# Ruslan361/iterative_solvers

Hardware: AMD Instinct MI355X
Metric: cg_iters_per_sec (higher is better)
Workload: dtype f64; 1 GPU; 4096x4096 L-shaped Dirichlet Poisson fp64, matrix-free CG, fixed 2641 iterations; n=4096, unknowns=12574721, rule=rel2

## Files before the change

### include/mi355cg.h

```cpp
#ifndef MI355CG_H
#define MI355CG_H

#include <stddef.h>

#ifdef __cplusplus
extern "C" {
#endif

#define MI355CG_OK            0
#define MI355CG_ERR_INVALID   1
#define MI355CG_ERR_HIP       2
#define MI355CG_ERR_STATE     3

#define MI355CG_F64           0
#define MI355CG_F32_MIXED     1

#define MI355CG_RULE_MSG_MAXNORM  0
#define MI355CG_RULE_REL_2NORM    1

#define MI355CG_STOP_ITERATIONS   0
#define MI355CG_STOP_PRECISION    1
#define MI355CG_STOP_RESIDUAL     2
#define MI355CG_STOP_EXACT_ERROR  3
#define MI355CG_STOP_INTERRUPTED  4
// ... 48 lines not shown
int  mi355cg_set_rhs(mi355cg_handle h, const double *b);
int  mi355cg_setup_on_device(mi355cg_handle h);

int  mi355cg_apply(mi355cg_handle h, const double *x, double *y);
int  mi355cg_apply_device(mi355cg_handle h, const double *x_dev, double *y_dev);

void mi355cg_default_params(mi355cg_params *p, int rule);
int  mi355cg_solve(mi355cg_handle h, const mi355cg_params *params,
                   mi355cg_iter_cb cb, void *user, const volatile int *stop_flag,
                   mi355cg_results *out);
int  mi355cg_get_solution(mi355cg_handle h, double *x);
int  mi355cg_get_recursive_residual(mi355cg_handle h, double *r);
int  mi355cg_get_true_residual(mi355cg_handle h, double *ax_minus_b);

#define MI355CG_PRECOND_NONE    0
#define MI355CG_PRECOND_MG      1
#define MI355CG_PRECOND_MG_ANY  2
int  mi355cg_set_preconditioner(mi355cg_handle h, int kind);
int  mi355cg_apply_preconditioner(mi355cg_handle h, const double *r, double *z);
int  mi355cg_mg_levels(int n, int *levels, int *coarsest_n);
int  mi355cg_mg_hierarchy(int kind, int n, int max_levels, int *levels, int *level_n);

#define MI355CG_CYCLE_F64 0
#define MI355CG_CYCLE_F32 1
int  mi355cg_set_preconditioner_ex(mi355cg_handle h, int kind, int cycle);
int  mi355cg_preconditioner_info(mi355cg_handle h, int *kind, int *cycle, int *levels);

#define MI355CG_SMOOTHER_JACOBI    0
#define MI355CG_SMOOTHER_LINE_X    1
#define MI355CG_SMOOTHER_LINE_Y    2
#define MI355CG_SMOOTHER_LINE_AUTO 3
int  mi355cg_set_smoother(mi355cg_handle h, int smoother);
int  mi355cg_get_smoother(mi355cg_handle h, int *smoother, int *direction);

#define MI355CG_BATCH_MAX 64
int  mi355cg_solve_batch(mi355cg_handle h, const mi355cg_params *params, int nrhs, const double *b, double *x,
                         const volatile int *stop_flag, mi355cg_results *out);
int  mi355cg_solve_batch_device(mi355cg_handle h, const mi355cg_params *params, int nrhs, const double *b_dev, double *x_dev,
                                const volatile int *stop_flag, mi355cg_results *out);
int  mi355cg_batch_release(mi355cg_handle h);

int  mi355cg_set_initial_guess(mi355cg_handle h, const double *x0);
int  mi355cg_set_initial_guess_device(mi355cg_handle h, const double *x0_dev);
int  mi355cg_use_solution_as_initial_guess(mi355cg_handle h);
int  mi355cg_solve_batch_from(mi355cg_handle h, const mi355cg_params *params, int nrhs, const double *b, double *x,
                              const volatile int *stop_flag, mi355cg_results *out);
int  mi355cg_solve_batch_device_from(mi355cg_handle h, const mi355cg_params *params, int nrhs, const double *b_dev, double *x_dev,
                                     const volatile int *stop_flag, mi355cg_results *out);

int  mi355cg_set_shift(mi355cg_handle h, double sigma);
int  mi355cg_get_shift(mi355cg_handle h, double *sigma);
int  mi355cg_time_steps(mi355cg_handle h, const mi355cg_params *params, double tau, double theta, int nsteps,
                        const volatile int *stop_flag, mi355cg_results *out , int *steps_done);
int  mi355cg_get_solution_device(mi355cg_handle h, double *x_dev);

#define MI355CG_EIG_BLOCK_MAX 16
#define MI355CG_EIG_CONVERGED   0
#define MI355CG_EIG_ITERATIONS  1
#define MI355CG_EIG_INTERRUPTED 2
#define MI355CG_EIG_BREAKDOWN   3
typedef struct mi355cg_eig_results {
    int iterations;
    int converged;
    int stop_reason;
    int p_drops;
    double solve_seconds;
} mi355cg_eig_results;
int  mi355cg_eigs(mi355cg_handle h, int nev, int block, double tol, int max_iterations, double *x, double *lambda, double *resid,
                  const volatile int *stop_flag, mi355cg_eig_results *out);
int  mi355cg_eigs_device(mi355cg_handle h, int nev, int block, double tol, int max_iterations, double *x_dev, double *lambda,
                         double *resid, const volatile int *stop_flag, mi355cg_eig_results *out);
int  mi355cg_eigs_release(mi355cg_handle h);
int  mi355cg_block_gram(mi355cg_handle h, int na, const double *a, int nb, const double *b, double *c);
int  mi355cg_block_gram_indexed(mi355cg_handle h, int na, const double *a, int nia, const int *ia, int nb, const double *b,
                                int nib, const int *ib, double *c);
int  mi355cg_block_combine(mi355cg_handle h, int k, const double *s, int m, const double *coef, double *y);
int  mi355cg_rayleigh_ritz(int k, const double *g, const double *hmat, double *theta, double *coef);

int  mi355cg_set_profiling(mi355cg_handle h, int enable);
int  mi355cg_get_kernel_time(mi355cg_handle h, int kernel, double *avg_ms, long long *launches);
int  mi355cg_get_layout(mi355cg_handle h, long long *padded_len, int *pitch_bottom, int *pitch_upper,
                        int *grid_stencil, int *grid_update, int *rows_per_item);
int  mi355cg_get_xfold(mi355cg_handle h, int *depth, int *extra_buffers);

#define MI355CG_SOLVE_LAUNCHES 0
#define MI355CG_SOLVE_ONCHIP   1
int  mi355cg_set_solve_mode(mi355cg_handle h, int mode);
int  mi355cg_get_solve_mode(mi355cg_handle h, int *mode, long long *onchip_launches_last_solve);
int  mi355cg_onchip_plan(int n, int *threads, int *lds_bytes, int *elems_per_thread);

#define MI355CG_MANY_MAX 65536
int  mi355cg_solve_many(mi355cg_handle h, const mi355cg_params *params, int nsys, const double *b, double *x, const double *sigma,
                        const volatile int *stop_flag, mi355cg_results *out);
int  mi355cg_solve_many_from(mi355cg_handle h, const mi355cg_params *params, int nsys, const double *b, double *x, const double *sigma,
                             const volatile int *stop_flag, mi355cg_results *out);
int  mi355cg_solve_many_device(mi355cg_handle h, const mi355cg_params *params, int nsys, const double *b_dev, double *x_dev,
                               const double *sigma_dev, const volatile int *stop_flag, mi355cg_results *out);
int  mi355cg_solve_many_device_from(mi355cg_handle h, const mi355cg_params *params, int nsys, const double *b_dev, double *x_dev,
                                    const double *sigma_dev, const volatile int *stop_flag, mi355cg_results *out);
int  mi355cg_solve_many_info(mi355cg_handle h, int nsys, int *lds_bytes_per_workgroup, int *workgroups_per_cu, long long *workspace_bytes);

int  mi355cg_slab_rows(int n, int world, int rank, int *y_lo, int *y_hi);
int  mi355cg_create_part(int n, int m, double a, double b, double c, double d, int dtype, int device,
                         int y_lo, int y_hi, int x_lo, int x_hi, mi355cg_handle *out);
int  mi355cg_checksum(mi355cg_handle h, int which, double *out2);
int  mi355cg_create_slab(int n, int m, double a, double b, double c, double d, int dtype, int device,
                         int y_lo, int y_hi, mi355cg_handle *out);
int  mi355cg_owned_range(mi355cg_handle h, long long *packed_begin, long long *packed_len, int *y_lo, int *y_hi);
int  mi355cg_dist_begin(mi355cg_handle h, const mi355cg_params *params, void *stream);
int  mi355cg_dist_reduce(mi355cg_handle h, int which , int with_rows, void *stream);
int  mi355cg_dist_sums_ptr(mi355cg_handle h, int which, void **dev_ptr, int *count );
int  mi355cg_dist_record_layout(mi355cg_handle h, int *header, int *row_slot, int *width);
int  mi355cg_dist_scatter_ghosts(mi355cg_handle h, int vector ,
                                 const double *gathered_records, int nranks, int rank, void *stream);
int  mi355cg_dist_stencil(mi355cg_handle h, const double *gathered_update_sums, int nranks, int estride,
                          int rows , void *stream);
int  mi355cg_dist_flip(mi355cg_handle h);
int  mi355cg_dist_update(mi355cg_handle h, const double *gathered_stencil_sums, int nranks, int estride,
                         int rows , void *stream);
int  mi355cg_dist_update_reads_ghosts(mi355cg_handle h);
int  mi355cg_dist_check(mi355cg_handle h, const double *gathered_update_sums, int nranks, int estride, void *stream);
int  mi355cg_dist_summary(mi355cg_handle h, mi355cg_results *out, int *done);
int  mi355cg_dist_finish(mi355cg_handle h, void *stream);
int  mi355cg_dist_history(mi355cg_handle h, int iteration, double *precision, double *residual, double *error);
int  mi355cg_dist_halo(mi355cg_handle h, int vector ,
                       void **send_lo, void **recv_lo, long long *n_send_lo,
                       void **send_hi, void **recv_hi, long long *n_send_hi);
int  mi355cg_dist_halo_recv_counts(mi355cg_handle h, long long *n_from_lo, long long *n_from_hi);

#define MI355CG_DECOMP_ROWS 0
#define MI355CG_DECOMP_2D   1
typedef struct mi355cg_team_s *mi355cg_team;
typedef struct mi355cg_halo_msg {
    int id;
    int peer;
    int send;
    int kind;
    int y0, y1, x0, x1;
    long long count;
} mi355cg_halo_msg;
int  mi355cg_decompose(int n, int world, int decomp, int rank, int *y_lo, int *y_hi, int *x_lo, int *x_hi);
int  mi355cg_halo_plan(int n, int world, int decomp, int rank, int max_msgs, int *n_msgs, mi355cg_halo_msg *msgs);
int  mi355cg_debug_plan(int n, int world, int decomp, int rank, int which, int *n_panels, int *panels,
                        int *grid, int *n_items, int *cls);
int  mi355cg_team_create_local(int n, int m, double a, double b, double c, double d, int world,
                               const int *devices, int ndevices, int decomp, mi355cg_team *out);
int  mi355cg_team_unique_id(void *id128);
int  mi355cg_team_create_rccl(int n, int m, double a, double b, double c, double d, int world, int rank, int device,
                              const void *id128, int decomp, mi355cg_team *out);
void mi355cg_team_destroy(mi355cg_team t);
int  mi355cg_team_solve(mi355cg_team t, const mi355cg_params *params, mi355cg_iter_cb cb, void *user,
                        const volatile int *stop_flag, mi355cg_results *out);
int  mi355cg_team_info(mi355cg_team t, int *world, int *nlocal, int *decomp, long long *size);
int  mi355cg_team_describe(mi355cg_team t, char *buf, int len);
int  mi355cg_team_part(mi355cg_team t, int local_index, mi355cg_handle *part, int *rank);
int  mi355cg_team_get_vector(mi355cg_team t, int which, double *global_packed);
int  mi355cg_team_checksum(mi355cg_team t, int which, double *out2);
int  mi355cg_team_set_vector(mi355cg_team t, int which, const double *global_packed);
int  mi355cg_team_set_dtype(mi355cg_team t, int dtype);
int  mi355cg_team_setup_on_device(mi355cg_team t);
int  mi355cg_team_set_profiling(mi355cg_team t, int enable);
int  mi355cg_team_phase_times(mi355cg_team t, double *kernel_ms, double *comm_ms, double *wall_ms);

#ifdef __cplusplus
}
#endif
// ... 2 lines not shown
```

### iterative_solvers_amd/_capi.py

```python
from __future__ import annotations

import ctypes as C
import os

import numpy as np

from . import build as _build

OK, ERR_INVALID, ERR_HIP, ERR_STATE = 0, 1, 2, 3
F64, F32_MIXED = 0, 1
RULE_MSG_MAXNORM, RULE_REL_2NORM = 0, 1
STOP_ITERATIONS, STOP_PRECISION, STOP_RESIDUAL, STOP_EXACT_ERROR, STOP_INTERRUPTED = range(5)

EXPORTS = [
    "mi355cg_create", "mi355cg_create_csr", "mi355cg_set_true_solution", "mi355cg_destroy", "mi355cg_last_error", "mi355cg_version", "mi355cg_size",
    "mi355cg_get_rhs", "mi355cg_get_true_solution", "mi355cg_get_node_coords", "mi355cg_set_rhs",
    "mi355cg_apply", "mi355cg_apply_device", "mi355cg_default_params", "mi355cg_solve",
    "mi355cg_get_solution", "mi355cg_get_recursive_residual", "mi355cg_get_true_residual",
    "mi355cg_set_profiling", "mi355cg_get_kernel_time", "mi355cg_get_layout",
    "mi355cg_slab_rows", "mi355cg_create_slab", "mi355cg_owned_range", "mi355cg_dist_begin",
    "mi355cg_dist_reduce", "mi355cg_dist_sums_ptr", "mi355cg_dist_record_layout", "mi355cg_dist_scatter_ghosts", "mi355cg_dist_stencil", "mi355cg_dist_flip",
    "mi355cg_dist_update", "mi355cg_dist_update_reads_ghosts", "mi355cg_dist_check", "mi355cg_dist_summary", "mi355cg_dist_finish", "mi355cg_dist_history",
    "mi355cg_dist_halo", "mi355cg_dist_halo_recv_counts",
    "mi355cg_create_part", "mi355cg_checksum", "mi355cg_decompose", "mi355cg_halo_plan",
    "mi355cg_team_create_local", "mi355cg_team_unique_id", "mi355cg_team_create_rccl", "mi355cg_team_destroy",
    "mi355cg_team_solve", "mi355cg_team_info", "mi355cg_team_part", "mi355cg_team_get_vector", "mi355cg_team_set_vector", "mi355cg_team_checksum",
    "mi355cg_team_set_profiling", "mi355cg_team_phase_times", "mi355cg_team_describe", "mi355cg_setup_on_device", "mi355cg_team_setup_on_device", "mi355cg_debug_plan",
    "mi355cg_team_set_dtype", "mi355cg_set_preconditioner", "mi355cg_apply_preconditioner", "mi355cg_mg_levels",
    "mi355cg_mg_hierarchy", "mi355cg_set_preconditioner_ex", "mi355cg_preconditioner_info",
    "mi355cg_solve_batch", "mi355cg_solve_batch_device", "mi355cg_batch_release", "mi355cg_get_xfold",
    "mi355cg_set_initial_guess", "mi355cg_set_initial_guess_device", "mi355cg_use_solution_as_initial_guess",
    "mi355cg_solve_batch_from", "mi355cg_solve_batch_device_from",
    "mi355cg_set_shift", "mi355cg_get_shift", "mi355cg_time_steps", "mi355cg_get_solution_device",
    "mi355cg_eigs", "mi355cg_eigs_device", "mi355cg_eigs_release", "mi355cg_block_gram", "mi355cg_block_gram_indexed",
    "mi355cg_block_combine", "mi355cg_rayleigh_ritz",
    "mi355cg_set_smoother", "mi355cg_get_smoother",
    "mi355cg_set_solve_mode", "mi355cg_get_solve_mode", "mi355cg_onchip_plan",
    "mi355cg_solve_many", "mi355cg_solve_many_from", "mi355cg_solve_many_device", "mi355cg_solve_many_device_from", "mi355cg_solve_many_info",
]
DECOMP_ROWS, DECOMP_2D = 0, 1
PRECOND_NONE, PRECOND_MG, PRECOND_MG_ANY = 0, 1, 2
CYCLE_F64, CYCLE_F32 = 0, 1
SOLVE_LAUNCHES, SOLVE_ONCHIP = 0, 1
SMOOTHER_JACOBI, SMOOTHER_LINE_X, SMOOTHER_LINE_Y, SMOOTHER_LINE_AUTO = 0, 1, 2, 3
BATCH_MAX = 64
MANY_MAX = 65536
EIG_BLOCK_MAX = 16
EIG_BASIS_MAX = 48
EIG_CONVERGED, EIG_ITERATIONS, EIG_INTERRUPTED, EIG_BREAKDOWN = range(4)


class Params(C.Structure):
    _fields_ = [("rule", C.c_int), ("max_iterations", C.c_int),
                ("eps_precision", C.c_double), ("eps_residual", C.c_double),
                ("eps_exact_error", C.c_double), ("eps_rel", C.c_double),
                ("use_true_solution", C.c_int), ("callback_every", C.c_int),
                ("diagnostics", C.c_int), ("sync_every", C.c_int), ("fixed_iterations", C.c_int),
                ("inner_eps", C.c_double)]


class Results(C.Structure):
    _fields_ = [("iterations", C.c_int), ("converged", C.c_int), ("stop_reason", C.c_int),
                ("final_residual_norm", C.c_double), ("final_precision", C.c_double),
                ("final_error_norm", C.c_double), ("r_norm2", C.c_double),
                ("initial_r_norm2", C.c_double), ("solve_seconds", C.c_double),
                ("refine_true_rel", C.c_double), ("refine_outer", C.c_int), ("loop_seconds", C.c_double)]


class EigResults(C.Structure):
    _fields_ = [("iterations", C.c_int), ("converged", C.c_int), ("stop_reason", C.c_int), ("p_drops", C.c_int),
                ("solve_seconds", C.c_double)]


class HaloMsg(C.Structure):
    _fields_ = [("id", C.c_int), ("peer", C.c_int), ("send", C.c_int), ("kind", C.c_int),
                ("y0", C.c_int), ("y1", C.c_int), ("x0", C.c_int), ("x1", C.c_int), ("count", C.c_longlong)]


ITER_CB = C.CFUNCTYPE(None, C.c_void_p, C.c_int, C.c_double, C.c_double, C.c_double)
_DP = np.ctypeslib.ndpointer(dtype=np.float64, flags="C_CONTIGUOUS")

_lib = None


class Mi355cgError(RuntimeError):
    def __init__(self, code: int, text: str):
        super().__init__(f"mi355cg error {code}: {text}")
        self.code = code


def lib_path() -> str:
    return _build.LIB_PATH


def load():
    global _lib
    if _lib is not None:
        return _lib
    path = os.environ.get("MI355CG_LIB") or _build.LIB_PATH
    if path == _build.LIB_PATH and _build.needs_build():
        try:
            _build.build()
        except Exception as e:
            if not os.path.exists(path):
                raise RuntimeError(f"libmi355cg.so is missing and could not be built: {e}") from e
    try:
        import torch
    except ImportError:
        pass
    L = C.CDLL(path)
    H = C.c_void_p
    L.mi355cg_create.argtypes = [C.c_int, C.c_int] + [C.c_double] * 4 + [C.c_int, C.c_int, C.POINTER(H)]
    _IPn = np.ctypeslib.ndpointer(dtype=np.int32, flags="C_CONTIGUOUS")
# ... 18 lines not shown
    L.mi355cg_get_kernel_time.argtypes = [H, C.c_int, C.POINTER(C.c_double), C.POINTER(C.c_longlong)]
    L.mi355cg_get_layout.argtypes = [H, C.POINTER(C.c_longlong)] + [C.POINTER(C.c_int)] * 5
    LLP, IP, VPP = C.POINTER(C.c_longlong), C.POINTER(C.c_int), C.POINTER(C.c_void_p)
    L.mi355cg_slab_rows.argtypes = [C.c_int, C.c_int, C.c_int, IP, IP]
    L.mi355cg_create_slab.argtypes = [C.c_int, C.c_int] + [C.c_double] * 4 + [C.c_int] * 4 + [C.POINTER(H)]
    L.mi355cg_owned_range.argtypes = [H, LLP, LLP, IP, IP]
    L.mi355cg_dist_begin.argtypes = [H, C.POINTER(Params), C.c_void_p]
    L.mi355cg_dist_reduce.argtypes = [H, C.c_int, C.c_int, C.c_void_p]
    L.mi355cg_dist_sums_ptr.argtypes = [H, C.c_int, VPP, IP]
    L.mi355cg_dist_record_layout.argtypes = [H, IP, IP, IP]
    L.mi355cg_dist_scatter_ghosts.argtypes = [H, C.c_int, C.c_void_p, C.c_int, C.c_int, C.c_void_p]
    L.mi355cg_dist_stencil.argtypes = [H, C.c_void_p, C.c_int, C.c_int, C.c_int, C.c_void_p]
    L.mi355cg_dist_flip.argtypes = [H]
    L.mi355cg_dist_update.argtypes = [H, C.c_void_p, C.c_int, C.c_int, C.c_int, C.c_void_p]
    L.mi355cg_dist_update_reads_ghosts.argtypes = [H]
    L.mi355cg_dist_check.argtypes = [H, C.c_void_p, C.c_int, C.c_int, C.c_void_p]
    L.mi355cg_dist_summary.argtypes = [H, C.POINTER(Results), IP]
    L.mi355cg_dist_finish.argtypes = [H, C.c_void_p]
    DBP = C.POINTER(C.c_double)
    L.mi355cg_dist_history.argtypes = [H, C.c_int, DBP, DBP, DBP]
    L.mi355cg_dist_halo.argtypes = [H, C.c_int, VPP, VPP, LLP, VPP, VPP, LLP]
    L.mi355cg_dist_halo_recv_counts.argtypes = [H, LLP, LLP]
    L.mi355cg_create_part.argtypes = [C.c_int, C.c_int] + [C.c_double] * 4 + [C.c_int] * 6 + [C.POINTER(H)]
    L.mi355cg_checksum.argtypes = [H, C.c_int, DBP]
    L.mi355cg_decompose.argtypes = [C.c_int] * 4 + [IP] * 4
    L.mi355cg_halo_plan.argtypes = [C.c_int] * 5 + [IP, C.POINTER(HaloMsg)]
    L.mi355cg_team_create_local.argtypes = [C.c_int, C.c_int] + [C.c_double] * 4 + [C.c_int, IP, C.c_int, C.c_int, C.POINTER(H)]
    L.mi355cg_team_unique_id.argtypes = [C.c_void_p]
    L.mi355cg_team_create_rccl.argtypes = [C.c_int, C.c_int] + [C.c_double] * 4 + [C.c_int, C.c_int, C.c_int, C.c_void_p, C.c_int, C.POINTER(H)]
    L.mi355cg_team_destroy.argtypes = [H]
    L.mi355cg_team_destroy.restype = None
    L.mi355cg_team_solve.argtypes = [H, C.POINTER(Params), ITER_CB, C.c_void_p, C.c_void_p, C.POINTER(Results)]
    L.mi355cg_team_info.argtypes = [H, IP, IP, IP, LLP]
    L.mi355cg_team_part.argtypes = [H, C.c_int, C.POINTER(H), IP]
    L.mi355cg_team_get_vector.argtypes = [H, C.c_int, _DP]
    L.mi355cg_team_set_vector.argtypes = [H, C.c_int, _DP]
    L.mi355cg_team_checksum.argtypes = [H, C.c_int, DBP]
    L.mi355cg_debug_plan.argtypes = [C.c_int] * 5 + [IP, IP, IP, IP, IP]
    L.mi355cg_setup_on_device.argtypes = [H]
    L.mi355cg_team_setup_on_device.argtypes = [H]
    L.mi355cg_team_set_dtype.argtypes = [H, C.c_int]
    L.mi355cg_team_set_profiling.argtypes = [H, C.c_int]
    L.mi355cg_team_phase_times.argtypes = [H, DBP, DBP, DBP]
    L.mi355cg_team_describe.argtypes = [H, C.c_char_p, C.c_int]
    L.mi355cg_set_preconditioner.argtypes = [H, C.c_int]
    L.mi355cg_set_preconditioner_ex.argtypes = [H, C.c_int, C.c_int]
    L.mi355cg_preconditioner_info.argtypes = [H, IP, IP, IP]
    L.mi355cg_apply_preconditioner.argtypes = [H, _DP, _DP]
    L.mi355cg_mg_levels.argtypes = [C.c_int, IP, IP]
    L.mi355cg_mg_hierarchy.argtypes = [C.c_int, C.c_int, C.c_int, IP, IP]
    L.mi355cg_solve_batch.argtypes = [H, C.POINTER(Params), C.c_int, C.c_void_p, C.c_void_p, C.c_void_p, C.POINTER(Results)]
    L.mi355cg_solve_batch_device.argtypes = [H, C.POINTER(Params), C.c_int, C.c_void_p, C.c_void_p, C.c_void_p, C.POINTER(Results)]
    L.mi355cg_batch_release.argtypes = [H]
    L.mi355cg_set_initial_guess.argtypes = [H, C.c_void_p]
    L.mi355cg_set_initial_guess_device.argtypes = [H, C.c_void_p]
    L.mi355cg_use_solution_as_initial_guess.argtypes = [H]
    L.mi355cg_solve_batch_from.argtypes = [H, C.POINTER(Params), C.c_int, C.c_void_p, C.c_void_p, C.c_void_p, C.POINTER(Results)]
    L.mi355cg_solve_batch_device_from.argtypes = [H, C.POINTER(Params), C.c_int, C.c_void_p, C.c_void_p, C.c_void_p, C.POINTER(Results)]
    L.mi355cg_set_shift.argtypes = [H, C.c_double]
    L.mi355cg_get_shift.argtypes = [H, DBP]
    L.mi355cg_time_steps.argtypes = [H, C.POINTER(Params), C.c_double, C.c_double, C.c_int, C.c_void_p, C.POINTER(Results), IP]
    L.mi355cg_get_solution_device.argtypes = [H, C.c_void_p]
    if hasattr(L, "mi355cg_eigs"):
        for fn in (L.mi355cg_eigs, L.mi355cg_eigs_device):
            fn.argtypes = [H, C.c_int, C.c_int, C.c_double, C.c_int, C.c_void_p, C.c_void_p, C.c_void_p, C.c_void_p, C.POINTER(EigResults)]
        L.mi355cg_eigs_release.argtypes = [H]
        L.mi355cg_block_gram.argtypes = [H, C.c_int, C.c_void_p, C.c_int, C.c_void_p, C.c_void_p]
        L.mi355cg_block_gram_indexed.argtypes = [H, C.c_int, C.c_void_p, C.c_int, C.c_void_p, C.c_int, C.c_void_p, C.c_int, C.c_void_p, C.c_void_p]
        L.mi355cg_block_combine.argtypes = [H, C.c_int, C.c_void_p, C.c_int, C.c_void_p, C.c_void_p]
        L.mi355cg_rayleigh_ritz.argtypes = [C.c_int, C.c_void_p, C.c_void_p, C.c_void_p, C.c_void_p]
    if hasattr(L, "mi355cg_set_smoother"):
        L.mi355cg_set_smoother.argtypes = [H, C.c_int]
        L.mi355cg_get_smoother.argtypes = [H, IP, IP]
    if hasattr(L, "mi355cg_set_solve_mode"):
        L.mi355cg_set_solve_mode.argtypes = [H, C.c_int]
        L.mi355cg_get_solve_mode.argtypes = [H, IP, LLP]
        L.mi355cg_onchip_plan.argtypes = [C.c_int, IP, IP, IP]
    if hasattr(L, "mi355cg_solve_many"):
        for fn in (L.mi355cg_solve_many, L.mi355cg_solve_many_from, L.mi355cg_solve_many_device, L.mi355cg_solve_many_device_from):
            fn.argtypes = [H, C.POINTER(Params), C.c_int, C.c_void_p, C.c_void_p, C.c_void_p, C.c_void_p, C.POINTER(Results)]
        L.mi355cg_solve_many_info.argtypes = [H, C.c_int, IP, IP, LLP]
    if hasattr(L, "mi355cg_get_xfold"):
        L.mi355cg_get_xfold.argtypes = [H, IP, IP]
    _lib = L
    return L


def check(rc: int):
    if rc != OK:
        raise Mi355cgError(rc, load().mi355cg_last_error().decode("utf-8", "replace"))
```

### iterative_solvers_amd/csrc/cg_kernels.h

```cpp
#pragma once
#include <hip/hip_runtime.h>
#include <cfloat>
#include <cmath>
#include "solve_loop.h"
#include "item_table.h"

namespace mi355cg {

#ifdef MI355CG_WAVE_TIMING
constexpr int kWtWaves = 16384, kWtStamps = 6;
__device__ unsigned long long g_wave_dbg[2][kWtStamps * kWtWaves];
#define MI355CG_WT_BEGIN unsigned long long wt_[kWtStamps]; for (int i_ = 0; i_ < kWtStamps; ++i_) wt_[i_] = 0; wt_[0] = wall_clock64();
#define MI355CG_WT_STAMP(I) wt_[I] = wall_clock64();
#define MI355CG_WT_MID wt_[kWtStamps - 2] = wall_clock64();
#define MI355CG_WT_END(K) do { if ((threadIdx.x & 63) == 0) { const int w_ = blockIdx.x * 4 + threadIdx.x / 64; \
    if (w_ < kWtWaves) { wt_[kWtStamps - 1] = wall_clock64(); for (int i_ = 0; i_ < kWtStamps; ++i_) g_wave_dbg[K][kWtStamps * w_ + i_] = wt_[i_]; } } } while (0)
#else
#define MI355CG_WT_BEGIN
#define MI355CG_WT_STAMP(I)
#define MI355CG_WT_MID
#define MI355CG_WT_END(K)
#endif

struct StateLite { double alpha, rr, rr_prev, rz, r0norm; int it, done, first, stop; };
// ... 436 lines not shown
__device__ inline rsrc_t make_rsrc(const void* base) {
    return __builtin_amdgcn_make_buffer_rsrc(const_cast<void*>(base), 0, 0x7fffffff, 0x00020000);
}
template <typename V> __device__ inline V buf_load(rsrc_t r, int voff, int soff) {
    if constexpr (sizeof(V) == 16) return __builtin_bit_cast(V, __builtin_amdgcn_raw_buffer_load_b128(r, voff, soff, 0));
    else if constexpr (sizeof(V) == 8) return __builtin_bit_cast(V, __builtin_amdgcn_raw_buffer_load_b64(r, voff, soff, 0));
    else { static_assert(sizeof(V) == 4, "buf_load: 4, 8 or 16 bytes"); return __builtin_bit_cast(V, __builtin_amdgcn_raw_buffer_load_b32(r, voff, soff, 0)); }
}
constexpr int kStPlain = 0, kStNt = 2, kStSc1 = 16;
template <int POLICY = kStPlain, typename V> __device__ inline void buf_store(V v, rsrc_t r, int voff, int soff) {
    typedef unsigned int u4 __attribute__((ext_vector_type(4)));
    typedef unsigned int u2 __attribute__((ext_vector_type(2)));
    if constexpr (sizeof(V) == 16) {
        u4 d = __builtin_bit_cast(u4, v);
        __builtin_amdgcn_raw_buffer_store_b128(d, r, voff, soff, POLICY);
        asm volatile("s_nop 1" : "+v"(d));
    }
    else if constexpr (sizeof(V) == 8) __builtin_amdgcn_raw_buffer_store_b64(__builtin_bit_cast(u2, v), r, voff, soff, POLICY);
    else { static_assert(sizeof(V) == 4, "buf_store: 4, 8 or 16 bytes"); __builtin_amdgcn_raw_buffer_store_b32(__builtin_bit_cast(unsigned int, v), r, voff, soff, POLICY); }
}
constexpr int kStorePnew = kStNt, kStoreR = kStSc1;
__device__ inline int dpp_from_below(int v) { return __builtin_amdgcn_update_dpp(0, v, 0x138 , 0xf, 0xf, false); }
__device__ inline int dpp_from_above(int v) { return __builtin_amdgcn_update_dpp(0, v, 0x130 , 0xf, 0xf, false); }
__device__ inline float lane_below(float v) { return __builtin_bit_cast(float, dpp_from_below(__builtin_bit_cast(int, v))); }
__device__ inline float lane_above(float v) { return __builtin_bit_cast(float, dpp_from_above(__builtin_bit_cast(int, v))); }
__device__ inline double lane_below(double v) {
    const unsigned long long u = __builtin_bit_cast(unsigned long long, v);
    const unsigned lo = (unsigned)dpp_from_below((int)(unsigned)u), hi = (unsigned)dpp_from_below((int)(unsigned)(u >> 32));
    return __builtin_bit_cast(double, ((unsigned long long)hi << 32) | lo);
}
__device__ inline double lane_above(double v) {
    const unsigned long long u = __builtin_bit_cast(unsigned long long, v);
    const unsigned lo = (unsigned)dpp_from_above((int)(unsigned)u), hi = (unsigned)dpp_from_above((int)(unsigned)(u >> 32));
    return __builtin_bit_cast(double, ((unsigned long long)hi << 32) | lo);
}
template <typename T> __device__ inline int row_step(const Geom& g, int y) { return (y + 1 <= g.half ? g.Pb : g.Pu) * (int)sizeof(T); }

template <typename T> __device__ inline int lane_off(const Geom& g, int x, bool bottom_row) {
    return (x < g.xlim && x >= (bottom_row ? g.cb : 0)) ? x * (int)sizeof(T) : kOob;
}
template <typename T, int VEC> __device__ inline int edge_off(const Geom& g, int x, int lane, bool bottom_row) {
    const int xe = lane == 0 ? x - 1 : x + VEC;
    const bool edge = lane == 0 || lane == kWave - 1;
    return (edge && xe >= (bottom_row ? g.cb : 0) && xe < g.xlim) ? xe * (int)sizeof(T) : kOob;
}

typedef ItemDesc Item;
__device__ inline Item decode_item(const ItemTab& t, int item) { return scalar_load16(t.items + item); }

__device__ inline int part_voff(int i, int n, int es) { return i < n ? i * es * (int)sizeof(double) : kOob; }
__device__ inline PreParts prefetch_parts_buf(rsrc_t rs, int field_off, int lo_off, int n, int es) {
    const int v0 = part_voff(threadIdx.x, n, es), v1 = part_voff(threadIdx.x + kBlock, n, es);
    PreParts p;
    p.hi0 = buf_load<double>(rs, v0, field_off); p.lo0 = buf_load<double>(rs, v0, field_off + lo_off);
    p.hi1 = buf_load<double>(rs, v1, field_off); p.lo1 = buf_load<double>(rs, v1, field_off + lo_off);
    return p;
}
__device__ inline PreMax prefetch_max_buf(rsrc_t rs, int field_off, int n, int es) {
    return PreMax{buf_load<double>(rs, part_voff(threadIdx.x, n, es), field_off), buf_load<double>(rs, part_voff(threadIdx.x + kBlock, n, es), field_off)};
}

struct ItemAddr {
    int nrows, ystart;
    long long base_el;
    int so_first, so_c0;
    int gc; bool bot;
    int x;
    int vo_own, ve_own, vo_first, vo_last;
};
template <typename T, int VEC, bool DESC>
__device__ inline ItemAddr item_addr(const Geom& g, const ItemUni& u, int lane) {
    constexpr int DIR = DESC ? -1 : 1;
    ItemAddr A;
    A.nrows = u.nrows; A.ystart = u.ystart; A.base_el = u.base_el; A.so_first = u.so_first; A.so_c0 = u.so_c0; A.gc = u.gc;
    A.bot = u.bot != 0;
    A.x = u.strip * (kWave * VEC) + lane * VEC;
    A.vo_own = lane_off<T>(g, A.x, A.bot);
    A.ve_own = edge_off<T, VEC>(g, A.x, lane, A.bot);
    A.vo_first = lane_off<T>(g, A.x, A.ystart - DIR <= g.half);
    A.vo_last = lane_off<T>(g, A.x, A.ystart + DIR * A.nrows <= g.half);
    return A;
}

template <typename T, int VEC, bool FUSED, bool MSG, int DEPTH, bool NOAP, bool GC, bool TEAM, bool QUEUE>
__global__ __launch_bounds__(kBlock) void k_stencil(const StencilArgs<T> a) {
    static_assert(DEPTH >= 1 && DEPTH <= 3, "the compute cursor takes its item from the fetch cursor: DEPTH <= rows fetched per item (>= 3)");
    typedef typename VecOf<T, VEC>::type vec_t;
    __shared__ double lds[2 * kWaves];
    const Geom& g = a.g;
    const int lane = threadIdx.x & (kWave - 1);
    const int wave = __builtin_amdgcn_readfirstlane(threadIdx.x / kWave);
    MI355CG_WT_BEGIN
    const StartRec rec = start_rec(a.tab.start, wave);
    const ItemSeq seq = rec.seq;
    struct Raw { vec_t r, p; T re, pe; };

    constexpr bool LEAN = FUSED && !TEAM;
    StateLite s_lean{};
    PreParts pre_lean{0.0, 0.0, 0.0, 0.0};
    PreMax pmax_lean[3] = {{0, 0}, {0, 0}, {0, 0}};
    if (LEAN) {
        s_lean = load_state_lite(a.s_in);
        const rsrc_t rs_part = make_rsrc(a.partB);
        const int fb = a.strideB * (int)sizeof(double);
        pre_lean = prefetch_parts_buf(rs_part, FB_RR * fb, FB_LO * fb, a.nB, a.esB);
        if (MSG) {
#pragma unroll
            for (int k = 0; k < 3; ++k) pmax_lean[k] = prefetch_max_buf(rs_part, (FB_RMAX + k) * fb, a.nB, a.esB);
        }
    }

    int f_item = seq.first;
    bool f_have = f_item < seq.end;
    ItemAddr F{};
    int f_idx = 0, f_so = 0, f_y = 0;
    rsrc_t rs_p = make_rsrc(a.pin), rs_r = make_rsrc(a.pin);
    const int dq_nsub = min(kQueueSubs, (int)(gridDim.x / kXcds)), dq_sub = (int)(blockIdx.x / kXcds) % dq_nsub;
    int* const dq = (QUEUE && a.dq.mine) ? a.dq.mine + ((int)(blockIdx.x % kXcds) * kQueueSubs + dq_sub) * kQueuePitch : nullptr;
    if (QUEUE && a.dq.other && blockIdx.x == 0 && threadIdx.x < kXcds * kQueueSubs) a.dq.other[threadIdx.x * kQueuePitch] = 0;
    int dq_ticket = 0;
    auto enter = [&](const ItemUni& u) {
        if (QUEUE && dq) dq_ticket = queue_take(dq, lane);
        F = item_addr<T, VEC, false>(g, u, lane);
        rs_p = make_rsrc(a.pin + F.base_el);
        rs_r = make_rsrc(FUSED ? a.r + F.base_el : a.pin + F.base_el);
        f_idx = -1; f_so = F.so_first; f_y = F.ystart - 1;
    };
    auto fetch = [&](bool may_switch = true) -> Raw {
        if (may_switch && f_have && f_idx > F.nrows) {
            f_item = (QUEUE && dq) ? seq.begin + seq.step + __builtin_amdgcn_readfirstlane(dq_ticket) * dq_nsub + dq_sub : f_item + seq.step;
            f_have = f_item < seq.end;
            if (f_have) enter(item_uniform<false>(g, decode_item(a.tab, f_item), (int)sizeof(T)));
        }
        const bool own = f_idx >= 0 && f_idx < F.nrows;
        int vo = own ? F.vo_own : (f_idx < 0 ? F.vo_first : F.vo_last);
        int ve = own ? F.ve_own : kOob;
        if (!f_have) { vo = kOob; ve = kOob; }
        Raw w;
        w.p = buf_load<vec_t>(rs_p, vo, f_so);
        if (FUSED) w.r = buf_load<vec_t>(rs_r, vo, f_so);
        else for (int j = 0; j < VEC; ++j) w.r[j] = (T)0;
        w.pe = buf_load<T>(rs_p, ve, f_so);
        if (FUSED) w.re = buf_load<T>(rs_r, ve, f_so); else w.re = (T)0;
        f_so += row_step<T>(g, f_y); ++f_y; ++f_idx;
        return w;
    };

    bool c_have = f_have;
    ItemAddr C{};
    int c_idx = -1, c_so = 0, c_y = 0, c_ve_gc = kOob;
    bool in_j[VEC];
#pragma unroll
    for (int j = 0; j < VEC; ++j) in_j[j] = false;
    rsrc_t rs_po = make_rsrc(a.pin), rs_ap = make_rsrc(a.pin);
    auto promote = [&]() {
        C = F;
        rs_po = make_rsrc(FUSED ? a.pout + C.base_el : a.pin + C.base_el);
        rs_ap = make_rsrc(NOAP ? a.pin + C.base_el : a.ap + C.base_el);
        c_idx = -1; c_so = C.so_c0; c_y = C.ystart;
        const int xint0 = C.bot ? g.half + 1 : 1;
#pragma unroll
        for (int j = 0; j < VEC; ++j) in_j[j] = (C.x + j >= xint0) && (C.x + j <= g.N - 1);
        if (GC) c_ve_gc = ((lane == 0 && (C.gc & 1)) || (lane == kWave - 1 && (C.gc & 2))) ? C.ve_own : kOob;
    };

    if (f_have) { enter(rec.u); promote(); }
    Raw q[DEPTH];
#pragma unroll
    for (int k = 0; k < DEPTH; ++k) q[k] = fetch(false);
    MI355CG_WT_STAMP(3)

    T beta = (T)0;
    if (LEAN) {
        const StateLite& s = s_lean;
        if (s.done) { if (blockIdx.x == 0 && threadIdx.x == 0) copy_state(a.s_out, a.s_in); return; }
        MI355CG_WT_STAMP(1)
        const Decision d = reduce_and_decide(s, a.rp, a.partB, a.nB, a.strideB, a.esB, a.want_diag, lds, &pre_lean, MSG ? pmax_lean : nullptr);
        MI355CG_WT_STAMP(2)
        if (blockIdx.x == 0 && threadIdx.x == 0) write_state_after_decision(a.s_out, a.hist, a.s_in, s, d);
        if (d.done) return;
        beta = (T)d.beta;
    } else if (FUSED && a.src.mbox) {
        __shared__ double recs[kMaxRecDst * kRecWords];
        const PreParts pre = prefetch_parts(a.partB + FB_RR * a.strideB, a.partB + (FB_RR + FB_LO) * a.strideB, a.nB, 1);
        PreMax pmax[3] = {{0, 0}, {0, 0}, {0, 0}};
        if (MSG) {
#pragma unroll
            for (int k = 0; k < 3; ++k) pmax[k] = prefetch_max(a.partB + (FB_RMAX + k) * a.strideB, a.nB, 1);
        }
        const StateLite s = load_state_lite(a.s_in);
        if (s.done) {
            if (threadIdx.x == 0) { store_flagged_zero(a.fl, a.slotA + blockIdx.x, FA_COUNT); if (blockIdx.x == 0) copy_state(a.s_out, a.s_in); }
            return;
        }
        MI355CG_WT_STAMP(1)
        own_record_B(recs, a.src.me, a.partB, a.nB, a.strideB, MSG ? 1 : 0, lds, &pre, MSG ? pmax : nullptr);
        if (!gather_records(a.src, recs)) {
            if (threadIdx.x == 0) { store_flagged_zero(a.fl, a.slotA + blockIdx.x, FA_COUNT); if (blockIdx.x == 0) fail_transport(a.s_out, a.s_in); }
            return;
        }
        const Decision d = decide_from_records(s, a.rp, recs, a.src.world, MSG, false);
        MI355CG_WT_STAMP(2)
        if (blockIdx.x == 0 && threadIdx.x == 0) write_state_after_decision(a.s_out, a.hist, a.s_in, s, d);
        if (d.done) { if (threadIdx.x == 0) store_flagged_zero(a.fl, a.slotA + blockIdx.x, FA_COUNT); return; }
        beta = (T)d.beta;
    } else if (FUSED) {
        const PreParts pre = prefetch_parts(a.partB + FB_RR * a.strideB, a.partB + (FB_RR + FB_LO) * a.strideB, a.nB, a.esB);
        PreMax pmax[3] = {{0, 0}, {0, 0}, {0, 0}};
        if (MSG) {
#pragma unroll
            for (int k = 0; k < 3; ++k) pmax[k] = prefetch_max(a.partB + (FB_RMAX + k) * a.strideB, a.nB, a.esB);
        }
        const StateLite s = load_state_lite(a.s_in);
        if (s.done) { if (blockIdx.x == 0 && threadIdx.x == 0) copy_state(a.s_out, a.s_in); return; }
        MI355CG_WT_STAMP(1)
        const Decision d = reduce_and_decide(s, a.rp, a.partB, a.nB, a.strideB, a.esB, a.want_diag, lds, &pre, MSG ? pmax : nullptr);
        MI355CG_WT_STAMP(2)
        if (blockIdx.x == 0 && threadIdx.x == 0) write_state_after_decision(a.s_out, a.hist, a.s_in, s, d);
        if (d.done) return;
        beta = (T)d.beta;
    }

    MI355CG_WT_MID
    const T cA = (T)g.A, cxk = (T)g.xk, cyk = (T)g.yk;
    dd acc_pap = dd_zero(), acc_rz = dd_zero();
// ... 150 lines not shown

    const dd t_rr = block_reduce_dd(s_rr, lds);
    const double t_rmax = block_reduce<true>(s_rmax, lds);
    const double t_dmax = block_reduce<true>(s_dmax, lds);
    const dd t_d2 = block_reduce_dd(s_d2, lds);
    double t_emax = 0; dd t_e2 = dd_zero();
    if (HAS_U) { t_emax = block_reduce<true>(s_emax, lds); t_e2 = block_reduce_dd(s_e2, lds); }
    if (threadIdx.x == 0) {
        const int b = blockIdx.x, st = a.strideB;
        a.partB[FB_RR * st + b] = t_rr.hi; a.partB[(FB_RR + FB_LO) * st + b] = t_rr.lo;
        a.partB[FB_D2 * st + b] = t_d2.hi; a.partB[(FB_D2 + FB_LO) * st + b] = t_d2.lo;
        a.partB[FB_E2 * st + b] = t_e2.hi; a.partB[(FB_E2 + FB_LO) * st + b] = t_e2.lo;
        a.partB[FB_RMAX * st + b] = t_rmax; a.partB[FB_DMAX * st + b] = t_dmax; a.partB[FB_EMAX * st + b] = t_emax;
        if (blockIdx.x == 0) {
            CgState* o = a.s_out;
            if (a.init == 1) {
                *o = CgState{};
                o->first = 1;
            } else {
                copy_state(a.s_out, a.s_in);
                if (a.init == 2) {
                    if (s.done) o->rr = s.rr_prev;
                    o->done = 0; o->reason = 0; o->converged = 0; o->alpha = 0.0; o->r0norm = a.r0norm_resume;
                    for (int i = 0; i < kRing; ++i) o->alpha_hist[i] = 0.0;
                } else { o->it = s.it + 1; o->first = 0; o->alpha = alpha_d; o->rz = rz; o->alpha_hist[(s.it + 1) & (kRing - 1)] = alpha_d; }
            }
        }
    }
}

template <typename T>
struct FreshArgs {
    long long begin, nvec;
    const T* b; T* x; T* r; T* p0; const T* u;
    double* partB; int strideB;
    CgState* s_out;
};
template <typename T, int VEC, bool HAS_U>
__global__ __launch_bounds__(kBlock) void k_init_fresh(const FreshArgs<T> a) {
    typedef typename VecOf<T, VEC>::type vec_t;
    __shared__ double lds[2 * kWaves];
    dd s_rr = dd_zero(), s_e2 = dd_zero();
    double s_rmax = 0, s_emax = 0;
    const long long stride = (long long)gridDim.x * kBlock;
    const vec_t* __restrict__ B = reinterpret_cast<const vec_t*>(a.b);
    const vec_t* __restrict__ Uu = reinterpret_cast<const vec_t*>(a.u);
    vec_t* __restrict__ X = reinterpret_cast<vec_t*>(a.x);
    vec_t* __restrict__ R = reinterpret_cast<vec_t*>(a.r);
    vec_t* __restrict__ P = reinterpret_cast<vec_t*>(a.p0);
    vec_t zero;
#pragma unroll
    for (int j = 0; j < VEC; ++j) zero[j] = (T)0;
    const long long end = a.begin + a.nvec;
    for (long long i = a.begin + (long long)blockIdx.x * kBlock + threadIdx.x; i < end; i += stride) {
        const vec_t bv = B[i];
        vec_t uv; if (HAS_U) uv = Uu[i];
#pragma unroll
        for (int j = 0; j < VEC; ++j) {
            const double rd = (double)bv[j];
            dd_acc_prod(s_rr, rd, rd);
            s_rmax = fmax(s_rmax, fabs(rd));
            if (HAS_U) {
                const double ee = (double)((T)0 - uv[j]);
                s_emax = fmax(s_emax, fabs(ee));
                dd_acc_prod(s_e2, ee, ee);
            }
        }
        X[i] = zero; R[i] = bv; P[i] = zero;
    }
    const dd t_rr = block_reduce_dd(s_rr, lds);
    const double t_rmax = block_reduce<true>(s_rmax, lds);
    double t_emax = 0; dd t_e2 = dd_zero();
    if (HAS_U) { t_emax = block_reduce<true>(s_emax, lds); t_e2 = block_reduce_dd(s_e2, lds); }
    if (threadIdx.x == 0) {
        const int b = blockIdx.x, st = a.strideB;
        a.partB[FB_RR * st + b] = t_rr.hi; a.partB[(FB_RR + FB_LO) * st + b] = t_rr.lo;
        a.partB[FB_D2 * st + b] = 0.0; a.partB[(FB_D2 + FB_LO) * st + b] = 0.0;
        a.partB[FB_E2 * st + b] = t_e2.hi; a.partB[(FB_E2 + FB_LO) * st + b] = t_e2.lo;
        a.partB[FB_RMAX * st + b] = t_rmax; a.partB[FB_DMAX * st + b] = 0.0; a.partB[FB_EMAX * st + b] = t_emax;
        if (blockIdx.x == 0) { *a.s_out = CgState{}; a.s_out->first = 1; }
    }
}

template <typename T>
struct GuessArgs {
    long long begin, nvec;
    const T* b; const T* ax; const T* x; T* r; T* p0; const T* u;
    double* partB; int strideB;
    double* partG; int strideG;
    CgState* s_out;
};
template <typename T, int VEC, bool HAS_U>
__global__ __launch_bounds__(kBlock) void k_init_guess(const GuessArgs<T> a) {
    typedef typename VecOf<T, VEC>::type vec_t;
    __shared__ double lds[2 * kWaves];
    dd s_rr = dd_zero(), s_bb = dd_zero(), s_e2 = dd_zero();
    double s_rmax = 0, s_emax = 0;
    const long long stride = (long long)gridDim.x * kBlock;
    const vec_t* __restrict__ B = reinterpret_cast<const vec_t*>(a.b);
    const vec_t* __restrict__ AX = reinterpret_cast<const vec_t*>(a.ax);
    const vec_t* __restrict__ X = reinterpret_cast<const vec_t*>(a.x);
    const vec_t* __restrict__ Uu = reinterpret_cast<const vec_t*>(a.u);
    vec_t* __restrict__ R = reinterpret_cast<vec_t*>(a.r);
    vec_t* __restrict__ P = reinterpret_cast<vec_t*>(a.p0);
    vec_t zero;
#pragma unroll
    for (int j = 0; j < VEC; ++j) zero[j] = (T)0;
    const long long end = a.begin + a.nvec;
    for (long long i = a.begin + (long long)blockIdx.x * kBlock + threadIdx.x; i < end; i += stride) {
        const vec_t bv = B[i], av = AX[i];
        vec_t xv, uv; if (HAS_U) { xv = X[i]; uv = Uu[i]; }
        vec_t rv;
#pragma unroll
        for (int j = 0; j < VEC; ++j) {
            rv[j] = bv[j] - av[j];
            const double rd = (double)rv[j], bd = (double)bv[j];
            dd_acc_prod(s_rr, rd, rd);
            dd_acc_prod(s_bb, bd, bd);
            s_rmax = fmax(s_rmax, fabs(rd));
            if (HAS_U) {
                const double ee = (double)(xv[j] - uv[j]);
                s_emax = fmax(s_emax, fabs(ee));
                dd_acc_prod(s_e2, ee, ee);
            }
        }
        R[i] = rv; P[i] = zero;
    }
    const dd t_rr = block_reduce_dd(s_rr, lds);
    const double t_rmax = block_reduce<true>(s_rmax, lds);
    double t_emax = 0; dd t_e2 = dd_zero();
    if (HAS_U) { t_emax = block_reduce<true>(s_emax, lds); t_e2 = block_reduce_dd(s_e2, lds); }
    const dd t_bb = block_reduce_dd(s_bb, lds);
    if (threadIdx.x == 0) {
        const int b = blockIdx.x, st = a.strideB;
        a.partB[FB_RR * st + b] = t_rr.hi; a.partB[(FB_RR + FB_LO) * st + b] = t_rr.lo;
        a.partB[FB_D2 * st + b] = 0.0; a.partB[(FB_D2 + FB_LO) * st + b] = 0.0;
        a.partB[FB_E2 * st + b] = t_e2.hi; a.partB[(FB_E2 + FB_LO) * st + b] = t_e2.lo;
        a.partB[FB_RMAX * st + b] = t_rmax; a.partB[FB_DMAX * st + b] = 0.0; a.partB[FB_EMAX * st + b] = t_emax;
        a.partG[b] = t_bb.hi; a.partG[a.strideG + b] = t_bb.lo;
        if (blockIdx.x == 0) { *a.s_out = CgState{}; a.s_out->first = 1; }
    }
}
__global__ __launch_bounds__(kBlock) void k_guess_state(const double* partB, int strideB, const double* partG, int strideG, int n,
                                                        CgState* s, double* norms) {
    __shared__ double lds[2 * kWaves];
    const double rr = dd_value(reduce_parts_dd(partB + FB_RR * strideB, partB + (FB_RR + FB_LO) * strideB, n, 1, lds));
    const double bb = dd_value(reduce_parts_dd(partG, partG + strideG, n, 1, lds));
    if (threadIdx.x == 0) { s->r0norm = sqrt(bb); s->first = 2; norms[0] = sqrt(rr); norms[1] = sqrt(bb); }
}

template <typename T>
struct UpdateStArgs {
    Geom g;
    ItemTab tab;
    const T* p;
    const T* pprev[kRing - 1];
    T* r; T* x; const T* u;
    const double* partA; int nA, strideA, esA;
    RecSrc src;
    double* partB; int strideB, slotB;
    const CgState* s_in; CgState* s_out;
    int rule;
    int reverse;
    const int* stop_req;
    FlagSpec fl;
    QueueSpec dq;
    double* fold_alpha;
    int fold_mask;
};

template <typename T, int VEC, int XM, bool HAS_U, int DEPTH, bool DESC, bool TEAM, bool QUEUE>
__global__ __launch_bounds__(kBlock) void k_update_st(const UpdateStArgs<T> a) {
    static_assert(DEPTH >= 1 && DEPTH <= 3, "see k_stencil");
    typedef typename VecOf<T, VEC>::type vec_t;
    __shared__ double lds[2 * kWaves];
    const Geom& g = a.g;
    const int lane = threadIdx.x & (kWave - 1);
    const int wave = __builtin_amdgcn_readfirstlane(threadIdx.x / kWave);
    MI355CG_WT_BEGIN
    const StartRec rec = start_rec(a.reverse ? a.tab.start_rev : a.tab.start, wave);
    const ItemSeq seq = rec.seq;
    constexpr bool FULL = XM == 1;
    constexpr int NP = XM >= 2 ? XM - 1 : 0;
    struct Raw { vec_t p, r, x, u, pp[NP > 0 ? NP : 1]; T pe; };

    StateLite s{};
    PreParts pre_lean{0.0, 0.0, 0.0, 0.0}, pre_rz_lean{0.0, 0.0, 0.0, 0.0};
    if (!TEAM) {
        s = load_state_lite(a.s_in);
        const rsrc_t rs_part = make_rsrc(a.partA);
        const int fa = a.strideA * (int)sizeof(double);
        pre_lean = prefetch_parts_buf(rs_part, FA_PAP * fa, FA_LO * fa, a.nA, a.esA);
        if (FULL) pre_rz_lean = prefetch_parts_buf(rs_part, FA_RZ * fa, FA_LO * fa, a.nA, a.esA);
    }

    int f_item = seq.first;
    bool f_have = f_item < seq.end;
    ItemAddr F{};
    int f_idx = 0, f_so = 0, f_y = 0;
    rsrc_t rs_p = make_rsrc(a.p), rs_r = rs_p, rs_x = rs_p, rs_u = rs_p;
    rsrc_t rs_pp[NP > 0 ? NP : 1] = {rs_p};
    const int dq_nsub = min(kQueueSubs, (int)(gridDim.x / kXcds)), dq_sub = (int)(blockIdx.x / kXcds) % dq_nsub;
    int* const dq = (QUEUE && a.dq.mine) ? a.dq.mine + ((int)(blockIdx.x % kXcds) * kQueueSubs + dq_sub) * kQueuePitch : nullptr;
    if (QUEUE && a.dq.other && blockIdx.x == 0 && threadIdx.x < kXcds * kQueueSubs) a.dq.other[threadIdx.x * kQueuePitch] = 0;
    int dq_ticket = 0;
    auto enter = [&](const ItemUni& u) {
        if (QUEUE && dq) dq_ticket = queue_take(dq, lane);
        F = item_addr<T, VEC, DESC>(g, u, lane);
        rs_p = make_rsrc(a.p + F.base_el);
        rs_r = make_rsrc(a.r + F.base_el);
        rs_x = make_rsrc(XM != 0 ? a.x + F.base_el : a.p + F.base_el);
#pragma unroll
        for (int i = 0; i < NP; ++i) rs_pp[i] = make_rsrc(a.pprev[i] + F.base_el);
        rs_u = make_rsrc((FULL && HAS_U) ? a.u + F.base_el : a.p + F.base_el);
        f_idx = -1; f_so = F.so_first; f_y = DESC ? F.ystart + 1 : F.ystart - 1;
    };
    auto fetch = [&](bool may_switch = true) -> Raw {
        if (may_switch && f_have && f_idx > F.nrows) {
            f_item = (QUEUE && dq) ? seq.begin + seq.step + __builtin_amdgcn_readfirstlane(dq_ticket) * dq_nsub + dq_sub : f_item + seq.step;
            f_have = f_item < seq.end;
            if (f_have) enter(item_uniform<DESC>(g, decode_item(a.tab, a.reverse ? seq.end - 1 - (f_item - seq.begin) : f_item), (int)sizeof(T)));
        }
        const bool own = f_have && f_idx >= 0 && f_idx < F.nrows;
        int vo = own ? F.vo_own : (f_idx < 0 ? F.vo_first : F.vo_last);
        if (!f_have) vo = kOob;
        const int vown = own ? F.vo_own : kOob;
        Raw w;
        w.p = buf_load<vec_t>(rs_p, vo, f_so);
        w.r = buf_load<vec_t>(rs_r, vown, f_so);
        if (XM != 0) w.x = buf_load<vec_t>(rs_x, vown, f_so);
#pragma unroll
        for (int i = 0; i < NP; ++i) w.pp[i] = buf_load<vec_t>(rs_pp[i], vown, f_so);
        if (FULL && HAS_U) w.u = buf_load<vec_t>(rs_u, vown, f_so);
        w.pe = buf_load<T>(rs_p, own ? F.ve_own : kOob, f_so);
        if (DESC) { f_so -= row_step<T>(g, f_y - 1); --f_y; } else { f_so += row_step<T>(g, f_y); ++f_y; }
        ++f_idx;
        return w;
    };

    bool c_have = f_have;
    ItemAddr C{};
    int c_idx = -1, c_so = 0, c_y = 0;
    bool in_j[VEC];
#pragma unroll
    for (int j = 0; j < VEC; ++j) in_j[j] = false;
    rsrc_t rs_ro = rs_p, rs_xo = rs_p;
    auto promote = [&]() {
        C = F;
        rs_ro = make_rsrc(a.r + C.base_el);
        rs_xo = make_rsrc(XM != 0 ? a.x + C.base_el : a.p + C.base_el);
        c_idx = -1; c_so = C.so_c0; c_y = C.ystart;
        const int xint0 = C.bot ? g.half + 1 : 1;
#pragma unroll
        for (int j = 0; j < VEC; ++j) in_j[j] = (C.x + j >= xint0) && (C.x + j <= g.N - 1);
    };

    if (f_have) { enter(rec.u); promote(); }
    Raw q[DEPTH];
#pragma unroll
    for (int k = 0; k < DEPTH; ++k) q[k] = fetch(false);
    MI355CG_WT_STAMP(3)
    int stop_word = 0;
    if (blockIdx.x == 0 && a.stop_req) stop_word = scalar_load(a.stop_req);

    double alpha_d, rz = 0.0;
    if (!TEAM) {
        if (s.done) { if (blockIdx.x == 0 && threadIdx.x == 0) copy_state(a.s_out, a.s_in); return; }
        MI355CG_WT_STAMP(1)
        const double pap = dd_value(reduce_parts_dd_pre(pre_lean, a.partA + FA_PAP * a.strideA, a.partA + (FA_PAP + FA_LO) * a.strideA, a.nA, a.esA, lds));
        if (a.rule == 0) {
            rz = FULL ? dd_value(reduce_parts_dd_pre(pre_rz_lean, a.partA + FA_RZ * a.strideA, a.partA + (FA_RZ + FA_LO) * a.strideA, a.nA, a.esA, lds))
                      : dd_value(reduce_parts_dd(a.partA + FA_RZ * a.strideA, a.partA + (FA_RZ + FA_LO) * a.strideA, a.nA, a.esA, lds));
            alpha_d = rz / pap;
        } else {
            alpha_d = s.rr / pap;
        }
        MI355CG_WT_STAMP(2)
    } else if (a.src.mbox) {
        __shared__ double recs[kMaxRecDst * kRecWords];
        const PreParts pre = prefetch_parts(a.partA + FA_PAP * a.strideA, a.partA + (FA_PAP + FA_LO) * a.strideA, a.nA, 1);
        PreParts pre_rz{0, 0, 0, 0};
        if (FULL) pre_rz = prefetch_parts(a.partA + FA_RZ * a.strideA, a.partA + (FA_RZ + FA_LO) * a.strideA, a.nA, 1);
        s = load_state_lite(a.s_in);
        if (s.done) {
            if (threadIdx.x == 0) { store_flagged_zero(a.fl, a.slotB + blockIdx.x, FB_LL_COUNT); if (blockIdx.x == 0) copy_state(a.s_out, a.s_in); }
            return;
        }
        {
            double* R = recs + a.src.me * kRecWords;
            if (threadIdx.x < kRecWords) R[threadIdx.x] = 0.0;
            const dd pap = reduce_parts_dd_pre(pre, a.partA + FA_PAP * a.strideA, a.partA + (FA_PAP + FA_LO) * a.strideA, a.nA, 1, lds);
            dd rzd = dd_zero();
            if (a.rule == 0) rzd = FULL ? reduce_parts_dd_pre(pre_rz, a.partA + FA_RZ * a.strideA, a.partA + (FA_RZ + FA_LO) * a.strideA, a.nA, 1, lds)
// ... 93 lines not shown
                }
                if (c_idx == C.nrows) {
                    c_have = f_have;
                    if (c_have) promote();
                } else ++c_idx;
            }
        }
    }

    MI355CG_WT_END(1);
    const dd t_rr = block_reduce_dd(s_rr, lds);
    const double t_rmax = block_reduce<true>(s_rmax, lds);
    double t_dmax = 0, t_emax = 0; dd t_d2 = dd_zero(), t_e2 = dd_zero();
    if (FULL) { t_dmax = block_reduce<true>(s_dmax, lds); t_d2 = block_reduce_dd(s_d2, lds); }
    if (FULL && HAS_U) { t_emax = block_reduce<true>(s_emax, lds); t_e2 = block_reduce_dd(s_e2, lds); }
    if (threadIdx.x == 0) {
        const int b = a.slotB + blockIdx.x, st = a.strideB;
        a.partB[FB_RR * st + b] = t_rr.hi; a.partB[(FB_RR + FB_LO) * st + b] = t_rr.lo;
        a.partB[FB_D2 * st + b] = t_d2.hi; a.partB[(FB_D2 + FB_LO) * st + b] = t_d2.lo;
        a.partB[FB_E2 * st + b] = t_e2.hi; a.partB[(FB_E2 + FB_LO) * st + b] = t_e2.lo;
        a.partB[FB_RMAX * st + b] = t_rmax; a.partB[FB_DMAX * st + b] = t_dmax; a.partB[FB_EMAX * st + b] = t_emax;
        if (TEAM && a.fl.part) {
            const double v[FB_LL_COUNT] = {t_rr.hi, t_d2.hi, t_e2.hi, t_rr.lo, t_d2.lo, t_e2.lo, t_rmax, t_dmax, t_emax, (blockIdx.x == 0 && stop_word) ? 1.0 : 0.0};
            store_flagged(a.fl, b, FB_LL_COUNT, v);
        }
        if (blockIdx.x == 0) {
            copy_state(a.s_out, a.s_in);
            CgState* o = a.s_out;
            o->it = s.it + 1; o->first = 0; o->alpha = alpha_d; o->rz = rz; o->alpha_hist[(s.it + 1) & (kRing - 1)] = alpha_d;
            o->stop = stop_word != 0;
            if (a.fold_alpha) a.fold_alpha[(s.it + 1) & a.fold_mask] = alpha_d;
        }
    }
}

struct CheckArgs {
    const double* partB; int nB, strideB, esB;
    RecSrc src;
    const CgState* s_in;
    CgState* summary;
    HistEntry* hist;
    RuleParams rp;
    int want_diag;
};
__global__ __launch_bounds__(kBlock) void k_check(const CheckArgs a) {
    __shared__ double lds[2 * kWaves];
    const StateLite s = load_state_lite(a.s_in);
    if (s.done) { if (threadIdx.x == 0) copy_state(a.summary, a.s_in); return; }
    Decision d;
    if (a.src.mbox) {
        __shared__ double recs[kMaxRecDst * kRecWords];
        own_record_B(recs, a.src.me, a.partB, a.nB, a.strideB, 2, lds);
        if (!gather_records(a.src, recs)) { if (threadIdx.x == 0) fail_transport(a.summary, a.s_in); return; }
        d = decide_from_records(s, a.rp, recs, a.src.world, true, true);
    } else d = reduce_and_decide(s, a.rp, a.partB, a.nB, a.strideB, a.esB, 1, lds);
    if (threadIdx.x == 0) write_state_after_decision(a.summary, a.hist, a.s_in, s, d);
}

template <typename T> struct FlushArgs { const T* p[kRing - 1]; T a[kRing - 1]; int n; };
template <typename T, int VEC>
__global__ __launch_bounds__(kBlock) void k_flush_x(const Geom g, const ItemTab tab, T* x, const FlushArgs<T> f) {
    typedef typename VecOf<T, VEC>::type vec_t;
    const int lane = threadIdx.x & (kWave - 1);
    const int wave = __builtin_amdgcn_readfirstlane(threadIdx.x / kWave);
    for (int item = blockIdx.x * kWaves + wave; item < tab.nitems; item += gridDim.x * kWaves) {
        const Item it = decode_item(tab, item);
        const int x0 = it.strip * (kWave * VEC) + lane * VEC;
        if (x0 < (it.ya <= g.half ? g.cb : 0) || x0 >= g.xlim) continue;
        for (int y = it.ya; y <= it.yb; ++y) {
            const long long off = row_off(g, y) - g.base0 + x0;
            vec_t xn = *reinterpret_cast<const vec_t*>(x + off);
#pragma unroll
            for (int k = 0; k < kRing - 1; ++k) if (k < f.n) {
                const vec_t pv = *reinterpret_cast<const vec_t*>(f.p[k] + off);
#pragma unroll
                for (int j = 0; j < VEC; ++j) xn[j] = xn[j] + f.a[k] * pv[j];
            }
            *reinterpret_cast<vec_t*>(x + off) = xn;
        }
    }
}

constexpr int kFoldMax = 32;
struct FoldTable { const double* p[kFoldMax]; double alpha[kFoldMax]; };
struct FoldArgs {
    long long begin, nvec;
    double* x;
    const FoldTable* tab;
    const CgState* s;
    int mask;
    int flush_it;
};
template <int NS, bool NT>
__device__ inline void fold_block(VecOf<double, 2>::type& xv, const FoldTable* tab, int k0, int mask, long long i) {
    typedef VecOf<double, 2>::type vec_t;
    const vec_t* P[NS]; double al[NS]; vec_t v[NS];
#pragma unroll
    for (int j = 0; j < NS; ++j) {
        const int slot = (k0 + j) & mask;
        P[j] = reinterpret_cast<const vec_t*>(scalar_load(&tab->p[slot]));
        al[j] = scalar_load(&tab->alpha[slot]);
    }
#pragma unroll
    for (int j = 0; j < NS; ++j) v[j] = NT ? __builtin_nontemporal_load(P[j] + i) : P[j][i];
#pragma unroll
    for (int j = 0; j < NS; ++j) { xv[0] = xv[0] + al[j] * v[j][0]; xv[1] = xv[1] + al[j] * v[j][1]; }
}
template <bool NT>
__global__ __launch_bounds__(kBlock) void k_fold_x(const FoldArgs a) {
    typedef VecOf<double, 2>::type vec_t;
    const int it = a.flush_it >= 0 ? a.flush_it : scalar_load(&a.s->it);
    int n = it & a.mask;
    if (a.flush_it < 0) {
        if (scalar_load(&a.s->done) || n != 0 || it == 0) return;
        n = a.mask + 1;
    }
    if (n == 0) return;
    vec_t* __restrict__ X = reinterpret_cast<vec_t*>(a.x);
    const long long stride = (long long)gridDim.x * kBlock, end = a.begin + a.nvec;
    for (long long i = a.begin + (long long)blockIdx.x * kBlock + threadIdx.x; i < end; i += stride) {
        vec_t xv = X[i];
        int k = it - n + 1;
        for (; k + 8 <= it + 1; k += 8) fold_block<8, NT>(xv, a.tab, k, a.mask, i);
        if (k + 4 <= it + 1) { fold_block<4, NT>(xv, a.tab, k, a.mask, i); k += 4; }
        if (k + 2 <= it + 1) { fold_block<2, NT>(xv, a.tab, k, a.mask, i); k += 2; }
        if (k <= it) fold_block<1, NT>(xv, a.tab, k, a.mask, i);
        X[i] = xv;
    }
}

template <typename T, int VEC>
__global__ __launch_bounds__(kBlock) void k_checksum(const Geom g, const ItemTab tab, const T* v, double* part) {
    typedef typename VecOf<T, VEC>::type vec_t;
    __shared__ double lds[2 * kWaves];
    const int lane = threadIdx.x & (kWave - 1);
    const int wave = __builtin_amdgcn_readfirstlane(threadIdx.x / kWave);
    dd s1 = dd_zero(), s2 = dd_zero();
    for (int item = blockIdx.x * kWaves + wave; item < tab.nitems; item += gridDim.x * kWaves) {
        const Item it = decode_item(tab, item);
        const int x0 = it.strip * (kWave * VEC) + lane * VEC;
        if (x0 < (it.ya <= g.half ? g.cb : 0) || x0 >= g.xlim) continue;
        for (int y = it.ya; y <= it.yb; ++y) {
            const vec_t t = *reinterpret_cast<const vec_t*>(v + (row_off(g, y) - g.base0 + x0));
#pragma unroll
            for (int j = 0; j < VEC; ++j) { s1 = dd_add(s1, dd{(double)t[j], 0.0}); dd_acc_prod(s2, (double)t[j], (double)t[j]); }
        }
    }
    const dd t1 = block_reduce_dd(s1, lds), t2 = block_reduce_dd(s2, lds);
    if (threadIdx.x == 0) {
        const int n = gridDim.x, b = blockIdx.x;
        part[b] = t1.hi; part[n + b] = t1.lo; part[2 * n + b] = t2.hi; part[3 * n + b] = t2.lo;
    }
}

template <typename T>
__global__ __launch_bounds__(kBlock) void k_err_maxnorm(long long begin, long long len, const T* x, const T* u, double* part) {
    __shared__ double lds[2 * kWaves];
    const long long stride = (long long)gridDim.x * kBlock;
    double m = 0.0;
    for (long long i = begin + (long long)blockIdx.x * kBlock + threadIdx.x; i < begin + len; i += stride)
        m = fmax(m, fabs((double)(x[i] - u[i])));
    const double t = block_reduce<true>(m, lds);
    if (threadIdx.x == 0) part[blockIdx.x] = t;
}

__global__ __launch_bounds__(kBlock) void k_residual_to_f32(long long total, long long own_begin, long long own_len,
                                                           const double* b, const double* ax, float* rf, double* part) {
    __shared__ double lds[2 * kWaves];
    const long long stride = (long long)gridDim.x * kBlock;
    double s = 0.0;
    for (long long i = (long long)blockIdx.x * kBlock + threadIdx.x; i < total; i += stride) {
        const double d = b[i] - ax[i];
        rf[i] = (float)d;
        if (i >= own_begin && i < own_begin + own_len) s += d * d;
    }
    const double t = block_reduce<false>(s, lds);
    if (threadIdx.x == 0) part[blockIdx.x] = t;
}
__global__ __launch_bounds__(kBlock) void k_accumulate_f32(long long begin, long long len, double* x, const float* d) {
    const long long stride = (long long)gridDim.x * kBlock;
    for (long long i = begin + (long long)blockIdx.x * kBlock + threadIdx.x; i < begin + len; i += stride) x[i] += (double)d[i];
}

struct RecordArgs {
    const double* part; int n, stride;
    int nsum, lo_off;
    int max_first, nmax;
    double* rec; int header, row_slot;
    const double* v; long long off_lo, off_hi; int len_lo, len_hi;
};
__global__ __launch_bounds__(kBlock) void k_make_record(const RecordArgs a) {
    __shared__ double lds[2 * kWaves];
    if (blockIdx.x == 0) {
        for (int f = 0; f < a.nsum; ++f) {
            const dd t = reduce_parts_dd(a.part + f * a.stride, a.part + (f + a.lo_off) * a.stride, a.n, 1, lds);
            if (threadIdx.x == 0) { a.rec[f] = t.hi; a.rec[f + a.lo_off] = t.lo; }
        }
        for (int f = a.max_first; f < a.max_first + a.nmax; ++f) {
            const double t = reduce_parts<true>(a.part + f * a.stride, a.n, 1, lds);
            if (threadIdx.x == 0) a.rec[f] = t;
        }
        return;
    }
    if (!a.v) return;
// ... 90 lines not shown
```

### iterative_solvers_amd/csrc/mi355cg.hip

```cpp
#include "../../include/mi355cg.h"
#include "cg_kernels.h"
#include "device_buffer.h"
#include "csr_kernels.h"
#include "grid_setup.h"
#include "mg_kernels.h"
#include "mg_batch_kernels.h"
#include "eig_kernels.h"
#include "mg_line_kernels.h"
#include "mg_kernels_f32.h"
#include "step_kernels.h"
#include "onchip_kernels.h"

#include <algorithm>
#include <cfloat>
#include <chrono>
#include <cstdarg>
#include <cstddef>
#include <cstdint>
#include <cstdio>
#include <cstdlib>
#include <cstring>
#include <memory>
#include <string>
#include <thread>
#include <vector>

using namespace mi355cg;

namespace {

thread_local std::string g_err;

int fail(int code, const char* fmt, ...) {
    char buf[512];
    va_list ap; va_start(ap, fmt); vsnprintf(buf, sizeof buf, fmt, ap); va_end(ap);
    g_err = buf;
    return code;
}

#define HIPCK(expr)                                                                                  \
    do {                                                                                             \
        hipError_t e_ = (expr);                                                                      \
        if (e_ != hipSuccess)                                                                        \
            return fail(MI355CG_ERR_HIP, "%s failed: %s (%s:%d)", #expr, hipGetErrorString(e_), __FILE__, __LINE__); \
    } while (0)

}

namespace mi355cg {
int mem_device_alloc(void** out, size_t bytes, bool zero, const char* what) {
    void* p = nullptr;
    hipError_t e = hipMalloc(&p, bytes);
    if (e == hipSuccess && zero && (e = hipMemset(p, 0, bytes)) != hipSuccess) hipFree(p);
    if (e == hipSuccess) { *out = p; return MI355CG_OK; }
    (void)hipGetLastError();
    return what ? fail(MI355CG_ERR_HIP, "%s", what) : fail(MI355CG_ERR_HIP, "device allocation of %zu bytes failed: %s", bytes, hipGetErrorString(e));
}
void mem_device_free(void* p) { if (p) hipFree(p); }
int mem_pinned_alloc(void** out, size_t bytes, const char* what) {
    void* p = nullptr;
    const hipError_t e = hipHostMalloc(&p, bytes);
    if (e == hipSuccess) { *out = p; return MI355CG_OK; }
    (void)hipGetLastError();
    return what ? fail(MI355CG_ERR_HIP, "%s", what) : fail(MI355CG_ERR_HIP, "pinned allocation of %zu bytes failed: %s", bytes, hipGetErrorString(e));
}
void mem_pinned_free(void* p) { if (p) hipHostFree(p); }
}

namespace {

int env_int(const char* name, int dflt) {
    const char* v = getenv(name);
    return (v && *v) ? atoi(v) : dflt;
}

inline long long round_up(long long v, long long m) { return (v + m - 1) / m * m; }

constexpr int kRecHeader = kRecWords;
constexpr int kStripCols = 128;

struct EventPool {
    std::vector<hipEvent_t> ev;
    size_t used = 0;
    hipEvent_t get() {
        if (used == ev.size()) { hipEvent_t e; if (hipEventCreate(&e) != hipSuccess) return nullptr; ev.push_back(e); }
        return ev[used++];
    }
    void reset() { used = 0; }
    void destroy() { for (auto e : ev) hipEventDestroy(e); ev.clear(); used = 0; }
};

struct MgLevel {
    Geom g{}; long long len = 0; int grid = 0; Buf<double> rhs, a, out;
    Buf<double> tab;
};
struct MgLevel32 { Buf<float> rhs, a, out; MgCoef32 c{}; float scale = 0.f; int vec = 1; };
struct MgHier {
    int kind = 0;
    int cycle = MI355CG_CYCLE_F64;
    int line_dir = 0;
    std::vector<MgLevel> lv;
    std::vector<MgLevel32> lv32;
    Buf<float> inv32;
    int ncoarse = 0;
    Buf<double> inv;
    Buf<int> coff;
    Buf<double> z, p[2], q;
// ... 27 lines not shown
    Buf<double> mat_h;
    Buf<double> red;
    Buf<double> stage;
};

struct OnchipManyWs {
    int cap = 0;
    Buf<double> vec;
    Buf<double> small;
    Buf<CgState> s, summary;
    Buf<int> done;
    Buf<CgState> summary_h;
    Buf<double> small_h;
    Buf<int> done_h;
    Buf<double> stage;
    long long stage_cap = 0;
};

}

struct mi355cg_ctx {
    int device = 0;
    int dtype = MI355CG_F64;
    hipStream_t stream = nullptr;
    GridParams gp;
    Geom g{};
    int s_lo = 0, s_hi = 0;
    long long storage_len = 0;
    long long pk_begin = 0, pk_len = 0;
    PackGeom pg{};
    Plan whole, interior, edge;
    Plan whole32;
    Buf<ItemDesc> plan_items[4];
    Buf<StartRec> plan_start[4][2];
    int depth = 2;
    bool has_gc = false;
    int nB_own = 0;
    int strideA = 0, strideB = 0;

    Buf<double> x, r, p[kRing], ap, b, u;
    int xsteps = 4;
    Buf<double> scratch[2];
    Buf<float> xf, rf, pf[kRing], apf;
    Buf<double> packed;
    Buf<double> partA, partB, partR;
    Buf<double> sumsA, sumsB;
    int rec_width = 0;
    mi355cg_params dist_prm{};
    bool dist_active = false, is_slab = false;
    Buf<CgState> sA, sB, summary;
    Buf<int> qctr;
    int dyn_rows = 0;
    Buf<int> stop_h;
    int* stop_dev = nullptr;
    Buf<HistEntry> hist;
    Buf<CgState> summary_h;
    Buf<HistEntry> hist_h;
    Buf<double> partR_h;

    std::vector<double> rhs_h, u_h;
    bool host_rhs_valid = true, host_u_valid = true;
    bool have_u_dev = false, solved = false;
    bool guess_pending = false;
    bool x_is_guess = false;
    Buf<double> guess_part;
    Buf<double> guess_norms_h;
    double sigma = 0.0;
    int smoother = MI355CG_SMOOTHER_JACOBI;
    Buf<double> step_b;
    bool is_csr = false;
    long long csr_n = 0, csr_nnz = 0;
    Buf<int> csr_row_map, csr_entries; Buf<double> csr_values;
    int grid_csr = 0, grid_update = 0;
    int cur = 0;
    int nA_dist = 0;
    int xfold = 0;
    double* fold_p[kFoldMax] = {};
    Buf<double> fold_own[kFoldMax];
    int fold_extra = 0;
    Buf<FoldTable> fold_tab;
    int fcur = 0;
    int fold_grid = 0;
    bool fold_nt = true;

    struct ChunkGraph { int m, cur; std::vector<char> flags; hipGraphExec_t exec; };
    std::vector<ChunkGraph> graphs;
    mi355cg_params graph_prm{};
    bool graph_stop = false;
    int use_graph = -1;
    int solve_mode = MI355CG_SOLVE_LAUNCHES;
    long long onchip_launches = 0;

    hipEvent_t ev_loop[2] = {nullptr, nullptr};
    std::unique_ptr<MgHier> mg;
    std::unique_ptr<MgBatchWs> batch;
    std::unique_ptr<EigWs> eig;
    std::unique_ptr<OnchipManyWs> many;
    bool profiling = false;
    EventPool events;
    std::vector<std::pair<hipEvent_t, hipEvent_t>> ev_pairs[2];
    double kernel_ms[2] = {0, 0};
    long long kernel_launches[2] = {0, 0};
};

namespace {

long long phys_start(const Geom& g, int y) { return row_off(g, y) + (y <= g.half ? g.cb : 0); }
long long phys_end(const Geom& g, int y) { return phys_start(g, y) + (y <= g.half ? g.Pb : g.Pu); }
int strips_total(const GridParams& gp, int vec) { return (gp.n - 1) / (kWave * vec) + 1; }
int first_bottom_strip(const GridParams& gp, int vec) { return (gp.half + 1) / (kWave * vec); }

void own_cols(const mi355cg_ctx* c, int y, int* xa, int* xb) {
    const int lo = y <= c->gp.half ? c->gp.half + 1 : 1, hi = c->gp.n;
    *xa = std::max(lo, c->s_lo * kStripCols);
    *xb = std::max(*xa, std::min(hi, c->s_hi * kStripCols));
}

void build_geom(mi355cg_ctx* c, int vec, int y_lo, int y_hi) {
    Geom& g = c->g;
    const GridParams& gp = c->gp;
    g.N = gp.n; g.half = gp.half;
    g.Pu = (int)round_up(g.N + 1, 32);
    g.cb = g.half & ~31;
    g.Pb = g.Pu - g.cb;
    g.xlim = (int)round_up(g.N + 1, vec);
    g.y_lo = y_lo; g.y_hi = y_hi;
    g.base0 = 0;
    g.base0 = phys_start(g, y_lo - 1);
    c->storage_len = phys_end(g, y_hi + 1) - g.base0;
    g.own_begin = phys_start(g, y_lo) - g.base0;
    g.own_len = phys_end(g, y_hi) - phys_start(g, y_lo);
    g.A = gp.A; g.xk = gp.x_k; g.yk = gp.y_k;
    PackGeom& pg = c->pg;
    pg.g = g;
    const int yb0 = y_lo, yb1 = std::min(y_hi, gp.half), yu0 = std::max(y_lo, gp.half + 1), yu1 = y_hi;
    int xa = 0, xb = 0;
    pg.nb_rows = std::max(0, yb1 - yb0 + 1); pg.yb0 = yb0;
    own_cols(c, gp.half, &xa, &xb); pg.xb0 = xa; pg.wb = pg.nb_rows ? xb - xa : 0;
    pg.nu_rows = std::max(0, yu1 - yu0 + 1); pg.yu0 = yu0;
    own_cols(c, gp.half + 1, &xa, &xb); pg.xu0 = xa; pg.wu = pg.nu_rows ? xb - xa : 0;
    pg.pk_len = (long long)pg.nb_rows * pg.wb + (long long)pg.nu_rows * pg.wu;
    c->pk_len = pg.pk_len;
    c->pk_begin = packed_row_begin(gp, y_lo);
}

int region_rects(const GridParams& gp, int vec, int ya, int yb, int sa, int sb, Rect out[2]) {
    const int ns_all = strips_total(gp, vec), s0b = first_bottom_strip(gp, vec);
    int nr = 0;
    sb = std::min(sb, ns_all);
    if (ya <= gp.half && yb >= 1) {
        const int s0 = std::max(sa, s0b);
        if (s0 < sb) out[nr++] = Rect{std::max(ya, 1), std::min(yb, gp.half), s0, sb, (sa > s0b ? 1 : 0) | (sb < ns_all ? 2 : 0)};
    }
    if (yb > gp.half && sa < sb)
        out[nr++] = Rect{std::max(ya, gp.half + 1), std::min(yb, gp.n - 1), sa, sb, (sa > 0 ? 1 : 0) | (sb < ns_all ? 2 : 0)};
    return nr;
}

PlanKnobs env_knobs() {
    PlanKnobs kn;
    kn.target_waves = env_int("MI355CG_WAVES", 2048); kn.max_blocks = env_int("MI355CG_BLOCKS", 512);
    { const char* v = getenv("MI355CG_ITEM_ROWS"); kn.item_rows = (v && *v) ? std::max(1, atoi(v)) : 0; }
    kn.xcd_classes = env_int("MI355CG_XCD_CLASSES", 1);
    return kn;
}
Plan make_plan(const std::vector<Rect>& rects, int max_rows, int fixed_ty = 0, int dyn_rows = 0) { return make_plan(rects, env_knobs(), max_rows, fixed_ty, dyn_rows); }
constexpr int kMaxRowsF64 = 800, kMaxRowsF32 = 64;

// ... 17 lines not shown
        const int si0 = r.s0 + ((r.gc & 1) ? 1 : 0), si1 = r.s1 - ((r.gc & 2) ? 1 : 0);
        if (r.y0 <= g.y_lo && g.y_lo <= r.y1) rows.push_back(Rect{g.y_lo, g.y_lo, r.s0, r.s1, r.gc});
        if (g.y_hi > g.y_lo && r.y0 <= g.y_hi && g.y_hi <= r.y1) rows.push_back(Rect{g.y_hi, g.y_hi, r.s0, r.s1, r.gc});
        if (yi0 > yi1) continue;
        if (si0 < si1) inner.push_back(Rect{yi0, yi1, si0, si1, 0});
        if (si0 >= si1) { cols.push_back(Rect{yi0, yi1, r.s0, r.s1, r.gc}); continue; }
        if (r.gc & 1) cols.push_back(Rect{yi0, yi1, r.s0, r.s0 + 1, 1});
        if (r.gc & 2) cols.push_back(Rect{yi0, yi1, r.s1 - 1, r.s1, 2});
    }
    c->interior = make_plan(inner, kMaxRowsF64);
    Plan e_rows = make_plan(rows, kMaxRowsF64, 1), e_cols = make_plan(cols, kMaxRowsF64, c->interior.ty > 0 ? c->interior.ty : 0);
    c->edge = e_rows;
    c->edge.wl.ncls = 1;
    for (int k = 0; k < e_cols.wl.np && c->edge.wl.np < kMaxPanels; ++k) {
        Panel P = e_cols.wl.p[k];
        P.item0 = c->edge.wl.nitems;
        c->edge.wl.p[c->edge.wl.np++] = P;
        c->edge.wl.nitems += P.ns * P.nchunks;
    }
    c->edge.grid = std::max(1, std::min(std::max(1, env_int("MI355CG_BLOCKS", 512)), (c->edge.wl.nitems + kWaves - 1) / kWaves));
    if (c->edge.wl.nitems == 0) c->edge.grid = 0;
    if (c->dtype == MI355CG_F32_MIXED || (c->s_lo == 0 && c->s_hi == strips_total(gp, 2))) {
        Rect r4[2];
        const int n4 = region_rects(gp, 4, g.y_lo, g.y_hi, 0, strips_total(gp, 4), r4);
        c->whole32 = make_plan(std::vector<Rect>(r4, r4 + n4), kMaxRowsF32);
    }
    c->depth = env_int("MI355CG_DEPTH", 3) == 2 ? 2 : 3;
    c->use_graph = env_int("MI355CG_GRAPH", -1);
    c->nB_own = c->whole.grid;
}

template <typename T>
int upload(const std::vector<T>& src, Buf<T>& dst, const char* what = nullptr) {
    Buf<T> fresh;
    if (int rc = Buf<T>::device(fresh, (long long)src.size(), what)) return rc;
    if (hipMemcpy(fresh, src.data(), sizeof(T) * src.size(), hipMemcpyHostToDevice) != hipSuccess) {
        const hipError_t e = hipGetLastError();
        return what ? fail(MI355CG_ERR_HIP, "%s", what) : fail(MI355CG_ERR_HIP, "upload of %zu bytes failed: %s", sizeof(T) * src.size(), hipGetErrorString(e));
    }
    dst = std::move(fresh);
    return MI355CG_OK;
}

int upload_item_tables(mi355cg_ctx* c) {
    int k = 0;
    for (Plan* pl : {&c->whole, &c->interior, &c->edge, &c->whole32}) {
        const int slot = k++;
        if (pl->wl.nitems == 0 || pl->grid == 0) continue;
        if (int rc = upload(build_item_table(pl->wl), c->plan_items[slot])) return rc;
        pl->d_items = c->plan_items[slot];
        pl->elem = pl == &c->whole32 ? (int)sizeof(float) : (int)sizeof(double);
        for (int rev = 0; rev < 2; ++rev) {
            if (int rc = upload(build_start_table(pl->wl, pl->grid, c->g, pl->elem, rev != 0), c->plan_start[slot][rev])) return rc;
            pl->d_start[rev] = c->plan_start[slot][rev];
        }
    }
    return MI355CG_OK;
}
ItemTab item_tab(const Plan& pl) { return ItemTab{pl.d_items, pl.d_start[0], pl.d_start[1], pl.wl.nitems}; }

int flat_grid(long long n) { return (int)std::max<long long>(1, std::min<long long>(2048, (n + kBlock - 1) / kBlock)); }

struct PartSrc { const double* ptr; int n, fstride, estride; RecSrc rec; };
struct Where { hipStream_t stream; const Plan* plan; int slot; };

Where whole_part(const mi355cg_ctx* c) { return Where{c->stream, &c->whole, 0}; }
PartSrc own_partB(const mi355cg_ctx* c) { return PartSrc{c->partB, c->nB_own, c->strideB, 1}; }
PartSrc own_partA(const mi355cg_ctx* c) { return PartSrc{c->partA, c->whole.grid, c->strideA, 1}; }

template <typename T, int VEC> Geom kernel_geom(const mi355cg_ctx* c) { Geom g = c->g; g.xlim = (int)round_up(c->g.N + 1, VEC); return g; }

template <typename T, int VEC>
void launch_apply(const mi355cg_ctx* c, const T* v, T* out, const Where& w) {
    if (w.plan->wl.nitems == 0) return;
    StencilArgs<T> a{};
    a.g = kernel_geom<T, VEC>(c); a.tab = item_tab(*w.plan);
    a.pin = v; a.ap = out; a.partA = nullptr;
    hipLaunchKernelGGL((k_stencil<T, VEC, false, false, 2, false, false, false, false>), dim3(w.plan->grid), dim3(kBlock), 0, w.stream, a);
}

struct IterCfg { RuleParams rp; int want_diag; bool has_u; bool x2 = false; bool fold = false; };

template <typename T, int VEC>
void launch_iteration_stencil(mi355cg_ctx* c, const IterCfg& cfg, const T* r, const Buf<T> p[kRing], const Where& w, const PartSrc& pb, const FlagSpec* fl = nullptr) {
    if (w.plan->wl.nitems == 0) return;
    StencilArgs<T> a{};
    a.g = kernel_geom<T, VEC>(c); a.tab = item_tab(*w.plan);
    a.r = r; a.pin = p[c->cur]; a.pout = p[(c->cur + 1) % c->xsteps]; a.ap = nullptr;
    a.partB = pb.ptr; a.nB = pb.n; a.strideB = pb.fstride; a.esB = pb.estride; a.src = pb.rec;
    a.partA = c->partA; a.strideA = c->strideA; a.slotA = w.slot;
    a.s_in = c->sB; a.s_out = c->sA; a.hist = c->hist; a.rp = cfg.rp; a.want_diag = cfg.want_diag;
    a.store_ghosts = c->is_slab ? 1 : 0;
    if (fl) a.fl = *fl;
    if (VEC == 2 && c->dyn_rows > 0 && w.plan == &c->whole) a.dq = QueueSpec{c->qctr, c->qctr + kXcds * kQueueSubs * kQueuePitch};
    const dim3 grid(w.plan->grid), block(kBlock);
    const bool msg = cfg.rp.rule == MI355CG_RULE_MSG_MAXNORM, gc = c->has_gc, d3 = c->depth == 3;
    const bool team = pb.rec.mbox != nullptr || (fl && fl->part), queue = a.dq.mine != nullptr;
#define MI355CG_ST(MSG, D, GC) do { if (team) hipLaunchKernelGGL((k_stencil<T, VEC, true, MSG, D, true, GC, true, VEC == 2>), grid, block, 0, w.stream, a); \
                                    else if (VEC == 2 && queue) hipLaunchKernelGGL((k_stencil<T, VEC, true, MSG, D, true, GC, false, VEC == 2>), grid, block, 0, w.stream, a); \
                                    else hipLaunchKernelGGL((k_stencil<T, VEC, true, MSG, D, true, GC, false, false>), grid, block, 0, w.stream, a); } while (0)
    if constexpr (VEC == 2) {
        if (msg) { if (gc) { if (d3) MI355CG_ST(true, 3, true); else MI355CG_ST(true, 2, true); } else { if (d3) MI355CG_ST(true, 3, false); else MI355CG_ST(true, 2, false); } }
        else     { if (gc) { if (d3) MI355CG_ST(false, 3, true); else MI355CG_ST(false, 2, true); } else { if (d3) MI355CG_ST(false, 3, false); else MI355CG_ST(false, 2, false); } }
    } else {
        if (d3) MI355CG_ST(false, 3, false); else MI355CG_ST(false, 2, false);
    }
#undef MI355CG_ST
}

template <typename T, int VEC>
void launch_iteration_update(mi355cg_ctx* c, const IterCfg& cfg, T* x, T* r, const Buf<T> p[kRing], const T* u, const Where& w, const PartSrc& pa, const FlagSpec* fl = nullptr) {
    if (w.plan->wl.nitems == 0) return;
    UpdateStArgs<T> a{};
    a.g = kernel_geom<T, VEC>(c); a.tab = item_tab(*w.plan);
    a.p = p[c->cur]; a.r = r; a.x = x; a.u = u;
    for (int i = 0; i < kRing - 1; ++i) a.pprev[i] = p[(c->cur + 2 * kRing * c->xsteps - 1 - i) % c->xsteps];
    a.partA = pa.ptr; a.nA = pa.n; a.strideA = pa.fstride; a.esA = pa.estride; a.src = pa.rec;
    a.partB = c->partB; a.strideB = c->strideB; a.slotB = w.slot;
    a.s_in = c->sA; a.s_out = c->sB; a.rule = cfg.rp.rule; a.reverse = 1;
    if (fl) a.fl = *fl;
    if (VEC == 2 && c->dyn_rows > 0 && w.plan == &c->whole) a.dq = QueueSpec{c->qctr + kXcds * kQueueSubs * kQueuePitch, c->qctr};
    if (cfg.fold) { a.fold_alpha = reinterpret_cast<double*>(reinterpret_cast<char*>(c->fold_tab.get()) + offsetof(FoldTable, alpha)); a.fold_mask = c->xfold - 1; }
    a.stop_req = w.slot == 0 ? c->stop_dev : nullptr;
    const dim3 grid(w.plan->grid), block(kBlock);
    const bool d3 = c->depth == 3 && !(cfg.x2 && c->cur == 0 && c->xsteps == 8);
    const bool team = pa.rec.mbox != nullptr || (fl && fl->part), queue = a.dq.mine != nullptr;
#define MI355CG_UST_D(XM, HASU, D) do { if (team) hipLaunchKernelGGL((k_update_st<T, VEC, XM, HASU, D, true, true, VEC == 2>), grid, block, 0, w.stream, a); \
                                        else if (VEC == 2 && queue) hipLaunchKernelGGL((k_update_st<T, VEC, XM, HASU, D, true, false, VEC == 2>), grid, block, 0, w.stream, a); \
                                        else hipLaunchKernelGGL((k_update_st<T, VEC, XM, HASU, D, true, false, false>), grid, block, 0, w.stream, a); } while (0)
#define MI355CG_UST(XM, HASU) do { if (d3) MI355CG_UST_D(XM, HASU, 3); else MI355CG_UST_D(XM, HASU, 2); } while (0)
    if (cfg.x2) {
        if (c->cur != 0 || cfg.fold) MI355CG_UST(0, false); else if (c->xsteps == 8) MI355CG_UST(8, false); else if (c->xsteps == 4) MI355CG_UST(4, false); else MI355CG_UST(2, false);
    }
    else if constexpr (VEC == 2) { if (cfg.has_u) MI355CG_UST(1, true); else MI355CG_UST(1, false); }
#undef MI355CG_UST
#undef MI355CG_UST_D
}

template <typename T, int VEC>
void launch_update_flat(mi355cg_ctx* c, const IterCfg& cfg, T* x, T* r, const T* p, const T* ap, const T* u, hipStream_t stream,
                        int grid, double resume_r0norm = -1.0) {
    UpdateArgs<T> a{};
    a.begin = c->g.own_begin / VEC; a.nvec = c->g.own_len / VEC;
    a.x = x; a.r = r; a.p = p; a.ap = ap; a.u = u;
    a.partA = c->partA; a.nA = 0; a.strideA = c->strideA; a.esA = 1;
    a.partB = c->partB; a.strideB = c->strideB;
    a.s_in = c->sA; a.s_out = c->sB; a.rule = cfg.rp.rule; a.init = 1;
    if (resume_r0norm >= 0.0) { a.init = 2; a.r0norm_resume = resume_r0norm; a.s_in = c->sB; }
    if (cfg.has_u) hipLaunchKernelGGL((k_update<T, VEC, true>), dim3(grid), dim3(kBlock), 0, stream, a);
    else hipLaunchKernelGGL((k_update<T, VEC, false>), dim3(grid), dim3(kBlock), 0, stream, a);
}

template <typename T, int VEC>
void launch_flush_x(const mi355cg_ctx* c, const Plan& plan, T* x, const Buf<T> p[kRing], const CgState& fin, hipStream_t stream) {
    const int pending = fin.it % c->xsteps;
    if (plan.wl.nitems == 0 || pending == 0) return;
    FlushArgs<T> f{};
    f.n = pending;
    for (int j = 0; j < pending; ++j) { const int k = fin.it - pending + 1 + j; f.p[j] = p[k % c->xsteps]; f.a[j] = (T)fin.alpha_hist[k & (kRing - 1)]; }
    hipLaunchKernelGGL((k_flush_x<T, VEC>), dim3(std::max(1, std::min(1024, (plan.wl.nitems + kWaves - 1) / kWaves))), dim3(kBlock), 0, stream,
                       kernel_geom<T, VEC>(c), item_tab(plan), x, f);
}

void launch_fold_x(const mi355cg_ctx* c, int flush_it, hipStream_t stream) {
    FoldArgs a{};
    a.begin = c->g.own_begin / 2; a.nvec = c->g.own_len / 2;
    a.x = c->x; a.tab = c->fold_tab; a.s = c->sB; a.mask = c->xfold - 1; a.flush_it = flush_it;
    const long long one_shot = (a.nvec + kBlock - 1) / kBlock;
    const int grid = (int)std::max<long long>(1, c->fold_grid > 0 ? std::min<long long>(c->fold_grid, one_shot) : one_shot);
    if (c->fold_nt) hipLaunchKernelGGL((k_fold_x<true>), dim3(grid), dim3(kBlock), 0, stream, a);
    else hipLaunchKernelGGL((k_fold_x<false>), dim3(grid), dim3(kBlock), 0, stream, a);
}
void free_fold_ring(mi355cg_ctx* c) {
    for (int k = c->xsteps; k < kFoldMax; ++k) { c->fold_own[k].reset(); c->fold_p[k] = nullptr; }
    c->fold_tab.reset();
    c->fold_extra = 0;
}
bool ensure_fold_ring(mi355cg_ctx* c) {
    if (c->xfold == 0) return false;
    if (c->fold_tab) return true;
    const size_t bytes = sizeof(double) * (size_t)c->storage_len;
    bool ok = true;
    for (int k = 0; k < c->xfold && ok; ++k) {
        if (k < c->xsteps) { c->fold_p[k] = c->p[k]; continue; }
        ok = Buf<double>::device(c->fold_own[k], c->storage_len) == MI355CG_OK && hipMemsetAsync(c->fold_own[k], 0, bytes, c->stream) == hipSuccess;
        c->fold_p[k] = c->fold_own[k];
    }
    FoldTable t{};
    for (int k = 0; k < c->xfold; ++k) t.p[k] = c->fold_p[k];
    ok = ok && Buf<FoldTable>::device(c->fold_tab, 1) == MI355CG_OK &&
         hipMemcpyAsync(c->fold_tab, &t, sizeof t, hipMemcpyHostToDevice, c->stream) == hipSuccess && hipStreamSynchronize(c->stream) == hipSuccess;
    if (!ok) {
        (void)hipGetLastError();
        hipStreamSynchronize(c->stream);
        free_fold_ring(c);
        c->xfold = 0;
        return false;
    }
    c->fold_extra = c->xfold - c->xsteps;
    return true;
}

void launch_check(mi355cg_ctx* c, const IterCfg& cfg, hipStream_t stream, const PartSrc& pb) {
    CheckArgs a{};
    a.partB = pb.ptr; a.nB = pb.n; a.strideB = pb.fstride; a.esB = pb.estride; a.src = pb.rec;
    a.s_in = c->sB; a.summary = c->summary; a.hist = c->hist; a.rp = cfg.rp; a.want_diag = cfg.want_diag;
    hipLaunchKernelGGL(k_check, dim3(1), dim3(kBlock), 0, stream, a);
}

IterCfg make_cfg(const mi355cg_params* prm) {
    IterCfg cfg{};
    const bool msg = prm->rule == MI355CG_RULE_MSG_MAXNORM;
    cfg.rp.rule = prm->rule; cfg.rp.max_iterations = prm->max_iterations;
    cfg.rp.eps_precision = prm->eps_precision; cfg.rp.eps_residual = prm->eps_residual;
    cfg.rp.eps_exact_error = prm->eps_exact_error; cfg.rp.eps_rel = prm->eps_rel;
    cfg.rp.fixed_iterations = prm->fixed_iterations;
    const bool diag = !msg && prm->diagnostics;
    cfg.has_u = (msg && prm->use_true_solution) || diag;
    cfg.rp.use_u = cfg.has_u ? 1 : 0;
    cfg.want_diag = diag ? 1 : 0;
    cfg.x2 = !msg && !diag;
    return cfg;
}

template <typename T>
int upload_packed(mi355cg_ctx* c, const double* host_packed, T* storage) {
    if (c->is_csr) {
        HIPCK(hipMemcpyAsync(storage, host_packed, sizeof(double) * c->pk_len, hipMemcpyHostToDevice, c->stream));
        HIPCK(hipStreamSynchronize(c->stream));
        return MI355CG_OK;
    }
    if (c->is_slab) HIPCK(hipDeviceSynchronize());
    if (c->pk_len == 0) return MI355CG_OK;
    HIPCK(hipMemcpyAsync(c->packed, host_packed, sizeof(double) * c->pk_len, hipMemcpyHostToDevice, c->stream));
    hipLaunchKernelGGL((k_unpack<T>), dim3(flat_grid(c->pk_len)), dim3(kBlock), 0, c->stream, c->pg, c->packed, storage);
    HIPCK(hipGetLastError());
    HIPCK(hipStreamSynchronize(c->stream));
    return MI355CG_OK;
}
template <typename T>
int download_packed(mi355cg_ctx* c, const T* storage, double* host_packed) {
    if (c->is_csr) {
        HIPCK(hipMemcpyAsync(host_packed, storage, sizeof(double) * c->pk_len, hipMemcpyDeviceToHost, c->stream));
        HIPCK(hipStreamSynchronize(c->stream));
        return MI355CG_OK;
    }
    if (c->is_slab) HIPCK(hipDeviceSynchronize());
    if (c->pk_len == 0) return MI355CG_OK;
    hipLaunchKernelGGL((k_pack<T>), dim3(flat_grid(c->pk_len)), dim3(kBlock), 0, c->stream, c->pg, storage, c->packed);
    HIPCK(hipGetLastError());
    HIPCK(hipMemcpyAsync(host_packed, c->packed, sizeof(double) * c->pk_len, hipMemcpyDeviceToHost, c->stream));
    HIPCK(hipStreamSynchronize(c->stream));
    return MI355CG_OK;
}

int ensure_host_copies(mi355cg_ctx* c) {
    if (!c->host_rhs_valid) { c->rhs_h.resize(c->pk_len); if (int rc = download_packed<double>(c, c->b, c->rhs_h.data())) return rc; c->host_rhs_valid = true; }
    if (!c->host_u_valid) { c->u_h.resize(c->pk_len); if (int rc = download_packed<double>(c, c->u, c->u_h.data())) return rc; c->host_u_valid = true; }
    return MI355CG_OK;
}
int ensure_f32_vectors(mi355cg_ctx* c) {
    if (c->xsteps > 4) return fail(MI355CG_ERR_INVALID, "MI355CG_XSTEPS=8 is fp64 only");
    if (c->whole32.wl.nitems == 0) return fail(MI355CG_ERR_INVALID, "the fp32 kernels march 256-column strips: a part of a 2-D decomposition (cut on 128 columns) cannot run them; use row slabs");
    if (c->g.own_begin % 4 != 0 || c->g.own_len % 4 != 0) return fail(MI355CG_ERR_STATE, "a part's owned range is not a whole number of float4");
    Buf<float>* fv[] = {&c->xf, &c->apf, &c->pf[0], &c->pf[1], &c->pf[2], &c->pf[3]};
    for (int k = 0; k < 2 + c->xsteps; ++k)
        if (!*fv[k]) if (int rc = Buf<float>::device_zeroed(*fv[k], c->storage_len, "fp32 vector allocation failed")) return rc;
    HIPCK(hipDeviceSynchronize());
    return MI355CG_OK;
}

int ensure_u_on_device(mi355cg_ctx* c) {
    if (c->have_u_dev) return MI355CG_OK;
    if (!c->host_u_valid) return fail(MI355CG_ERR_STATE, "no exact solution on host or device");
    if (int rc = upload_packed<double>(c, c->u_h.data(), c->u)) return rc;
    c->have_u_dev = true;
    return MI355CG_OK;
}
int ensure_scratch(mi355cg_ctx* c) {
    for (auto& s : c->scratch) if (!s) { if (int rc = Buf<double>::device_zeroed(s, c->storage_len)) return rc; }
    HIPCK(hipDeviceSynchronize());
    return MI355CG_OK;
}

int ensure_guess_ws(mi355cg_ctx* c) {
    if (!c->guess_part) if (int rc = Buf<double>::device(c->guess_part, 2 * (long long)c->strideB + 2)) return rc;
    if (!c->guess_norms_h) if (int rc = Buf<double>::pinned(c->guess_norms_h, 2)) return rc;
    return MI355CG_OK;
}

void clear_graphs(mi355cg_ctx* c) {
    for (auto& g : c->graphs) hipGraphExecDestroy(g.exec);
    c->graphs.clear();
}

void prof_begin(mi355cg_ctx* c, hipEvent_t* e0) {
    if (!c->profiling) return;
    *e0 = c->events.get();
    if (*e0) hipEventRecord(*e0, c->stream);
}
void prof_end(mi355cg_ctx* c, int k, hipEvent_t e0) {
    if (!c->profiling || !e0) return;
    hipEvent_t e1 = c->events.get();
    if (!e1) return;
    hipEventRecord(e1, c->stream);
    c->ev_pairs[k].push_back({e0, e1});
}
void prof_collect(mi355cg_ctx* c) {
    for (int k = 0; k < 2; ++k) {
        double tot = 0; long long n = 0;
        for (auto& pr : c->ev_pairs[k]) {
            float ms = 0;
            if (hipEventElapsedTime(&ms, pr.first, pr.second) == hipSuccess) { tot += ms; ++n; }
        }
        c->kernel_ms[k] = n ? tot / n : 0.0;
        c->kernel_launches[k] = n;
        c->ev_pairs[k].clear();
    }
    c->events.reset();
}

int fetch_state(mi355cg_ctx* c, hipStream_t st) {
    HIPCK(hipMemcpyAsync(c->summary_h, c->summary, sizeof(CgState), hipMemcpyDeviceToHost, st));
    HIPCK(hipMemcpyAsync(c->hist_h, c->hist, sizeof(HistEntry) * kHist, hipMemcpyDeviceToHost, st));
    return MI355CG_OK;
}
int wait_stream_forwarding_stop(mi355cg_ctx* c, const volatile int* stop_flag) {
    if (!stop_flag) { HIPCK(hipStreamSynchronize(c->stream)); return MI355CG_OK; }
    for (;;) {
        if (*stop_flag) *c->stop_h = 1;
        const hipError_t q = hipStreamQuery(c->stream);
        if (q == hipSuccess) break;
        if (q != hipErrorNotReady) HIPCK(q);
        std::this_thread::yield();
    }
    return MI355CG_OK;
}
int loop_timer_begin(mi355cg_ctx* c, hipStream_t st) {
    if (!c->ev_loop[0]) { HIPCK(hipEventCreate(&c->ev_loop[0])); HIPCK(hipEventCreate(&c->ev_loop[1])); }
    HIPCK(hipEventRecord(c->ev_loop[0], st));
    return MI355CG_OK;
}
int loop_timer_end(mi355cg_ctx* c, hipStream_t st) { HIPCK(hipEventRecord(c->ev_loop[1], st)); return MI355CG_OK; }
double loop_timer_seconds(const mi355cg_ctx* c) {
    float ms = 0;
    return hipEventElapsedTime(&ms, c->ev_loop[0], c->ev_loop[1]) == hipSuccess ? 1e-3 * ms : 0.0;
}

}

namespace {

CsrView csr_view(const mi355cg_ctx* c) { return CsrView{c->csr_n, c->csr_row_map, c->csr_entries, c->csr_values}; }

void launch_csr_spmv(mi355cg_ctx* c, const double* x, double* y, const double* r, const CgState* s_in, double* partA) {
    SpmvArgs a{};
    a.A = csr_view(c); a.x = x; a.y = y; a.r = r; a.s_in = s_in; a.partA = partA; a.strideA = c->strideA;
    hipLaunchKernelGGL(k_csr_spmv, dim3(c->grid_csr), dim3(kBlock), 0, c->stream, a);
}

int solve_csr(mi355cg_ctx* c, const mi355cg_params* prm, mi355cg_iter_cb cb, void* user,
              const volatile int* stop_flag, mi355cg_results* out) {
    if (prm->diagnostics) return fail(MI355CG_ERR_INVALID, "per-iteration diagnostics are not available on CSR handles");
    const bool msg = prm->rule == MI355CG_RULE_MSG_MAXNORM;
    IterCfg cfg = make_cfg(prm);
    if (cfg.has_u && !c->have_u_dev) { cfg.has_u = false; cfg.rp.use_u = 0; }
    const auto t0 = std::chrono::steady_clock::now();
    const size_t bytes = sizeof(double) * c->storage_len;
    HIPCK(hipMemsetAsync(c->x, 0, bytes, c->stream));
    HIPCK(hipMemsetAsync(c->p[0], 0, bytes, c->stream));
    HIPCK(hipMemsetAsync(c->ap, 0, bytes, c->stream));
    HIPCK(hipMemcpyAsync(c->r, c->b, bytes, hipMemcpyDeviceToDevice, c->stream));
    c->cur = 0;
    const PartSrc pA{c->partA, c->grid_csr, c->strideA, 1};
    auto update = [&](bool init, bool with_u) {
        UpdateArgs<double> a{};
        a.begin = 0; a.nvec = c->csr_n;
        a.x = c->x; a.r = c->r; a.p = c->p[0]; a.ap = c->ap; a.u = c->u;
        a.partA = pA.ptr; a.nA = pA.n; a.strideA = pA.fstride; a.esA = 1;
        a.partB = c->partB; a.strideB = c->strideB;
        a.s_in = c->sA; a.s_out = c->sB; a.rule = cfg.rp.rule; a.init = init ? 1 : 0;
        if (with_u) hipLaunchKernelGGL((k_update<double, 1, true>), dim3(c->grid_update), dim3(kBlock), 0, c->stream, a);
        else hipLaunchKernelGGL((k_update<double, 1, false>), dim3(c->grid_update), dim3(kBlock), 0, c->stream, a);
    };
    update(true, cfg.has_u);
    HIPCK(hipGetLastError());
    auto poll = [&]() -> int {
        launch_check(c, cfg, c->stream, own_partB(c));
        if (int rc = fetch_state(c, c->stream)) return rc;
        HIPCK(hipStreamSynchronize(c->stream));
        return MI355CG_OK;
    };
    if (int rc = poll()) return rc;
    const double initial_rnorm2 = c->summary_h->rnorm2;
    if (msg && cb) cb(user, 0, DBL_MAX, c->summary_h->rmax, cfg.has_u ? c->summary_h->emax : DBL_MAX);
    const int sync_every = default_sync_every(prm, msg);
    int it_done = 0;
    bool first_chunk = (cb != nullptr || stop_flag != nullptr);
    bool interrupted = false;
    while (!c->summary_h->done) {
        if (stop_flag && *stop_flag) { interrupted = true; break; }
        const int m = chunk_len(prm, msg, sync_every, it_done, first_chunk);
        first_chunk = false;
        for (int k = 0; k < m; ++k) {
            XpayArgs xa{};
            xa.n = c->csr_n; xa.r = c->r; xa.p = c->p[0];
            xa.partB = c->partB; xa.nB = c->grid_update; xa.strideB = c->strideB; xa.esB = 1;
// ... 1059 lines not shown
        at += counts[s];
    }
    hipLaunchKernelGGL(k_mgb_unpack, dim3(flat_grid(c->pk_len), n), dim3(kBlock), 0, c->stream, c->pg, vlen, (const double*)T.packed, T.vec);
    HIPCK(hipGetLastError());
    return MI355CG_OK;
}

}

extern "C" {

const char* mi355cg_last_error(void) { return g_err.c_str(); }
const char* mi355cg_version(void) { return "mi355cg 0.2 (gfx950)"; }

static const char* onchip_refusal(const mi355cg_ctx* c) {
    static char buf[160];
    if (c->is_csr) return "the on-chip solve keeps the grid's direction in LDS: a CSR handle has no grid";
    if (c->is_slab) return "the on-chip solve is one workgroup on one GPU: this handle owns one part of a decomposed grid";
    if (c->dtype != MI355CG_F64) return "the on-chip solve is fp64 only: this handle was created with MI355CG_F32_MIXED";
    if (c->mg) return "the on-chip solve runs plain CG: this handle has a preconditioner (mi355cg_set_preconditioner(h, MI355CG_PRECOND_NONE) first)";
    if (!onchip_supported(c->gp.n)) {
        snprintf(buf, sizeof buf, "the on-chip solve takes grids up to N = %d (the direction must fit in one CU's LDS): this handle has N = %d", kOnchipMaxN, c->gp.n);
        return buf;
    }
    return nullptr;
}
static int create_state(mi355cg_ctx* c, const char* what) {
    if (int rc = Buf<double>::device_zeroed(c->partA, (long long)FA_COUNT * c->strideA)) return rc;
    if (int rc = Buf<double>::device_zeroed(c->partB, (long long)FB_COUNT * c->strideB)) return rc;
    if (int rc = Buf<double>::device_zeroed(c->partR, 2048)) return rc;
    for (Buf<CgState>* s : {&c->sA, &c->sB, &c->summary}) if (int rc = Buf<CgState>::device_zeroed(*s, 1, what)) return rc;
    if (int rc = Buf<HistEntry>::device_zeroed(c->hist, kHist, what)) return rc;
    if (int rc = Buf<CgState>::pinned(c->summary_h, 1, what)) return rc;
    if (int rc = Buf<HistEntry>::pinned(c->hist_h, kHist, what)) return rc;
    return Buf<double>::pinned(c->partR_h, 2048, what);
}

static int create_impl(int n, int m, double a, double b, double c_, double d, int dtype, int device,
                       int y_lo, int y_hi, int s_lo, int s_hi, bool part, mi355cg_handle* out) {
    if (!out) return fail(MI355CG_ERR_INVALID, "out is null");
    *out = nullptr;
    if (dtype != MI355CG_F64 && dtype != MI355CG_F32_MIXED) return fail(MI355CG_ERR_INVALID, "unknown dtype %d", dtype);
    GridParams gp;
    if (!grid_params_init(&gp, n, m, a, b, c_, d))
        return fail(MI355CG_ERR_INVALID, "grid %dx%d rejected: the L-shaped index map is only consistent for n == m, even, >= 6", n, m);
    int ndev = 0;
    if (hipGetDeviceCount(&ndev) != hipSuccess || ndev <= 0)
        return fail(MI355CG_ERR_HIP, "no HIP device available (libmi355cg has no CPU fallback)");
    if (device < 0 || device >= ndev) return fail(MI355CG_ERR_INVALID, "device %d out of range (0..%d)", device, ndev - 1);
    HIPCK(hipSetDevice(device));

    const int ns_all = strips_total(gp, 2);
    if (!part) { y_lo = 1; y_hi = gp.n - 1; s_lo = 0; s_hi = ns_all; }
    if (y_lo < 1 || y_hi > gp.n - 1 || y_lo > y_hi)
        return fail(MI355CG_ERR_INVALID, "part rows [%d, %d] outside 1..%d", y_lo, y_hi, gp.n - 1);
    if (s_lo < 0 || s_hi > ns_all || s_lo >= s_hi)
        return fail(MI355CG_ERR_INVALID, "part strips [%d, %d) outside 0..%d", s_lo, s_hi, ns_all);
    if (dtype == MI355CG_F32_MIXED && part) return fail(MI355CG_ERR_INVALID, "F32_MIXED is single-GPU only");
    mi355cg_ctx* c = new mi355cg_ctx();
    c->device = device; c->dtype = dtype; c->gp = gp; c->is_slab = part;
    c->s_lo = s_lo; c->s_hi = s_hi;
    build_geom(c, 2, y_lo, y_hi);
    build_plans(c);
    c->strideA = std::max({c->whole.grid, c->interior.grid + c->edge.grid, c->whole32.grid, 1});
    c->strideB = c->strideA;

    int rc = MI355CG_OK;
    auto cleanup = [&]() { mi355cg_destroy(c); return rc; };
    if (hipStreamCreateWithFlags(&c->stream, hipStreamNonBlocking) != hipSuccess) { rc = fail(MI355CG_ERR_HIP, "hipStreamCreate failed"); return cleanup(); }
    if ((rc = upload_item_tables(c))) return cleanup();
    const long long L = c->storage_len;
    { const int m = env_int("MI355CG_XSTEPS", 4); c->xsteps = m == 2 ? 2 : ((m == 8 && dtype == MI355CG_F64) ? 8 : 4); }
    if (!part && dtype == MI355CG_F64 && !getenv("MI355CG_XSTEPS")) {
        const char* xf = getenv("MI355CG_XFOLD");
        const int want = (xf && *xf) ? atoi(xf) : -1;
        if (want == 16 || want == 32) c->xfold = want;
        else if (want < 0 && c->g.own_len >= (4LL << 20)) {
            size_t mem_free = 0, mem_total = 0;
            if (hipMemGetInfo(&mem_free, &mem_total) == hipSuccess)
                for (int R : {32, 16}) if (c->xfold == 0 && sizeof(double) * (size_t)L * (size_t)R <= mem_total / 4) c->xfold = R;
        }
        c->fold_grid = std::max(0, env_int("MI355CG_XFOLD_GRID", 0));
        c->fold_nt = env_int("MI355CG_XFOLD_NT", 1) != 0;
    }
    Buf<double>* vecs[] = {&c->x, &c->r, &c->p[0], &c->p[1], &c->ap, &c->b, &c->u, &c->p[2], &c->p[3], &c->p[4], &c->p[5], &c->p[6], &c->p[7]};
    for (int k = 0; k < 7 + (c->xsteps - 2); ++k) if ((rc = Buf<double>::device_zeroed(*vecs[k], L))) return cleanup();
    if (dtype == MI355CG_F32_MIXED) {
        Buf<float>* fv[] = {&c->xf, &c->rf, &c->pf[0], &c->pf[1], &c->apf, &c->pf[2], &c->pf[3], &c->pf[4], &c->pf[5], &c->pf[6], &c->pf[7]};
        for (int k = 0; k < 5 + (c->xsteps - 2); ++k) if ((rc = Buf<float>::device_zeroed(*fv[k], L, "fp32 vector allocation failed"))) return cleanup();
    }
    if ((rc = Buf<double>::device_zeroed(c->packed, std::max<long long>(c->pk_len, 1)))) return cleanup();
    if ((rc = create_state(c, "state allocation failed"))) return cleanup();
    c->rec_width = kRecHeader + 2 * c->g.Pu;
    if ((rc = Buf<double>::device_zeroed(c->sumsA, c->rec_width))) return cleanup();
    if ((rc = Buf<double>::device_zeroed(c->sumsB, c->rec_width))) return cleanup();
    if ((rc = Buf<int>::device_zeroed(c->qctr, 2 * kXcds * kQueueSubs * kQueuePitch, "queue counter allocation failed"))) return cleanup();
    if ((rc = Buf<int>::pinned(c->stop_h, 1, "stop word allocation failed"))) return cleanup();
    *c->stop_h = 0;
    if (hipDeviceSynchronize() != hipSuccess) { rc = fail(MI355CG_ERR_HIP, "hipDeviceSynchronize failed"); return cleanup(); }

    if (env_int("MI355CG_DEVICE_SETUP", 0)) {
        c->host_rhs_valid = false; c->host_u_valid = false;
        if ((rc = mi355cg_setup_on_device(c))) return cleanup();
    } else {
        c->rhs_h.resize(c->pk_len); c->u_h.resize(c->pk_len);
        grid_fill_box(gp, c->g.y_lo, c->g.y_hi, s_lo * kStripCols, s_hi == ns_all ? gp.n : s_hi * kStripCols, c->rhs_h.data(), c->u_h.data(), nullptr, nullptr);
        if ((rc = upload_packed<double>(c, c->rhs_h.data(), c->b))) return cleanup();
    }
    if (env_int("MI355CG_ONCHIP", 0) == 1 && !onchip_refusal(c)) c->solve_mode = MI355CG_SOLVE_ONCHIP;
    *out = c;
    return MI355CG_OK;
}

int mi355cg_create(int n, int m, double a, double b, double c_, double d, int dtype, int device, mi355cg_handle* out) {
    return create_impl(n, m, a, b, c_, d, dtype, device, 0, 0, 0, 0, false, out);
}
int mi355cg_create_slab(int n, int m, double a, double b, double c_, double d, int dtype, int device,
                        int y_lo, int y_hi, mi355cg_handle* out) {
    GridParams gp;
    if (!grid_params_init(&gp, n, m, a, b, c_, d)) return fail(MI355CG_ERR_INVALID, "grid %dx%d rejected: the L-shaped index map is only consistent for n == m, even, >= 6", n, m);
    return create_impl(n, m, a, b, c_, d, dtype, device, y_lo, y_hi, 0, strips_total(gp, 2), true, out);
}
int mi355cg_create_part(int n, int m, double a, double b, double c_, double d, int dtype, int device,
                        int y_lo, int y_hi, int x_lo, int x_hi, mi355cg_handle* out) {
    GridParams gp;
    if (!grid_params_init(&gp, n, m, a, b, c_, d)) return fail(MI355CG_ERR_INVALID, "grid %dx%d rejected: the L-shaped index map is only consistent for n == m, even, >= 6", n, m);
    const int ns_all = strips_total(gp, 2);
    if (x_lo % kStripCols != 0 || (x_hi % kStripCols != 0 && x_hi < gp.n))
        return fail(MI355CG_ERR_INVALID, "part columns [%d, %d): x-cuts must be multiples of %d", x_lo, x_hi, kStripCols);
    return create_impl(n, m, a, b, c_, d, dtype, device, y_lo, y_hi, x_lo / kStripCols, x_hi >= gp.n ? ns_all : x_hi / kStripCols, true, out);
}

int mi355cg_create_csr(long long nrows, const int* row_map, const int* entries, const double* values,
                       int device, mi355cg_handle* out) {
    if (!out) return fail(MI355CG_ERR_INVALID, "out is null");
    *out = nullptr;
    if (nrows <= 0 || !row_map || !entries || !values) return fail(MI355CG_ERR_INVALID, "bad CSR arguments");
    if (row_map[0] != 0) return fail(MI355CG_ERR_INVALID, "row_map[0] must be 0");
    const long long nnz = row_map[nrows];
    for (long long i = 0; i < nrows; ++i) if (row_map[i + 1] < row_map[i]) return fail(MI355CG_ERR_INVALID, "row_map is not monotone at row %lld", i);
    for (long long j = 0; j < nnz; ++j) if (entries[j] < 0 || entries[j] >= nrows) return fail(MI355CG_ERR_INVALID, "column index %d out of range at entry %lld", entries[j], j);
    int ndev = 0;
    if (hipGetDeviceCount(&ndev) != hipSuccess || ndev <= 0) return fail(MI355CG_ERR_HIP, "no HIP device available (libmi355cg has no CPU fallback)");
    if (device < 0 || device >= ndev) return fail(MI355CG_ERR_INVALID, "device %d out of range (0..%d)", device, ndev - 1);
    HIPCK(hipSetDevice(device));
    mi355cg_ctx* c = new mi355cg_ctx();
    c->device = device; c->dtype = MI355CG_F64; c->is_csr = true;
    c->csr_n = nrows; c->csr_nnz = nnz;
    c->gp.size = nrows; c->pk_begin = 0; c->pk_len = nrows; c->storage_len = nrows; c->pg.pk_len = nrows;
    c->g.own_begin = 0; c->g.own_len = nrows;
    const long long nblk = (nrows + kBlock - 1) / kBlock;
    c->grid_csr = (int)std::max<long long>(1, std::min<long long>(2048, nblk));
    c->grid_update = (int)std::max<long long>(1, std::min<long long>(512, nblk));
    c->strideA = c->grid_csr; c->strideB = c->grid_update; c->nB_own = c->grid_update;
    int rc = MI355CG_OK;
    auto cleanup = [&]() { mi355cg_destroy(c); return rc; };
    if (hipStreamCreateWithFlags(&c->stream, hipStreamNonBlocking) != hipSuccess) { rc = fail(MI355CG_ERR_HIP, "hipStreamCreate failed"); return cleanup(); }
    for (Buf<double>* v : {&c->x, &c->r, &c->p[0], &c->p[1], &c->ap, &c->b, &c->u}) if ((rc = Buf<double>::device_zeroed(*v, nrows))) return cleanup();
    if ((rc = create_state(c, "allocation failed"))) return cleanup();
    if ((rc = Buf<int>::device(c->csr_row_map, nrows + 1, "allocation failed")) || (rc = Buf<int>::device(c->csr_entries, std::max<long long>(nnz, 1), "allocation failed")) ||
        (rc = Buf<double>::device(c->csr_values, std::max<long long>(nnz, 1), "allocation failed"))) return cleanup();
    if (hipMemcpy(c->csr_row_map, row_map, sizeof(int) * (nrows + 1), hipMemcpyHostToDevice) != hipSuccess ||
        hipMemcpy(c->csr_entries, entries, sizeof(int) * nnz, hipMemcpyHostToDevice) != hipSuccess ||
        hipMemcpy(c->csr_values, values, sizeof(double) * nnz, hipMemcpyHostToDevice) != hipSuccess) {
        rc = fail(MI355CG_ERR_HIP, "CSR upload failed"); return cleanup();
    }
// ... 61 lines not shown
    HIPCK(hipGetLastError());
    HIPCK(hipStreamSynchronize(c->stream));
    c->have_u_dev = true; c->host_rhs_valid = false; c->host_u_valid = false;
    return MI355CG_OK;
}
int mi355cg_set_rhs(mi355cg_handle c, const double* b) {
    if (!c || !b) return fail(MI355CG_ERR_INVALID, "null argument");
    HIPCK(hipSetDevice(c->device));
    c->host_rhs_valid = true;
    c->rhs_h.resize(c->pk_len);
    std::memcpy(c->rhs_h.data(), b, sizeof(double) * c->pk_len);
    return upload_packed<double>(c, c->rhs_h.data(), c->b);
}

int mi355cg_apply_device(mi355cg_handle c, const double* x_dev, double* y_dev) {
    if (!c || !x_dev || !y_dev) return fail(MI355CG_ERR_INVALID, "null argument");
    if (c->is_slab) return fail(MI355CG_ERR_STATE, "this handle owns one part of a decomposed grid: use the mi355cg_team_* / mi355cg_dist_* entry points");
    HIPCK(hipSetDevice(c->device));
    if (c->is_csr) {
        launch_csr_spmv(c, x_dev, y_dev, nullptr, nullptr, nullptr);
        HIPCK(hipGetLastError());
        HIPCK(hipStreamSynchronize(c->stream));
        return MI355CG_OK;
    }
    if (int rc = ensure_scratch(c)) return rc;
    hipLaunchKernelGGL((k_unpack<double>), dim3(flat_grid(c->pk_len)), dim3(kBlock), 0, c->stream, c->pg, x_dev, c->scratch[0]);
    launch_apply<double, 2>(c, c->scratch[0], c->scratch[1], whole_part(c));
    hipLaunchKernelGGL((k_pack<double>), dim3(flat_grid(c->pk_len)), dim3(kBlock), 0, c->stream, c->pg, c->scratch[1], y_dev);
    HIPCK(hipGetLastError());
    HIPCK(hipStreamSynchronize(c->stream));
    return MI355CG_OK;
}

int mi355cg_apply(mi355cg_handle c, const double* x, double* y) {
    if (!c || !x || !y) return fail(MI355CG_ERR_INVALID, "null argument");
    if (c->is_slab) return fail(MI355CG_ERR_STATE, "this handle owns one part of a decomposed grid: use the mi355cg_team_* / mi355cg_dist_* entry points");
    HIPCK(hipSetDevice(c->device));
    if (int rc = ensure_scratch(c)) return rc;
    if (int rc = upload_packed<double>(c, x, c->scratch[0])) return rc;
    if (c->is_csr) launch_csr_spmv(c, c->scratch[0], c->scratch[1], nullptr, nullptr, nullptr);
    else launch_apply<double, 2>(c, c->scratch[0], c->scratch[1], whole_part(c));
    HIPCK(hipGetLastError());
    return download_packed<double>(c, c->scratch[1], y);
}

void mi355cg_default_params(mi355cg_params* p, int rule) {
    if (!p) return;
    std::memset(p, 0, sizeof *p);
    p->rule = rule;
    p->max_iterations = 10000;
    p->eps_precision = 1e-6; p->eps_residual = 1e-6; p->eps_exact_error = 1e-6;
    p->eps_rel = 1e-6;
    p->use_true_solution = 1;
    p->callback_every = rule == MI355CG_RULE_MSG_MAXNORM ? 100 : 1;
    p->diagnostics = 0;
    p->sync_every = 0;
    p->fixed_iterations = 0;
    p->inner_eps = 0.0;
}

static int launch_init_guess(mi355cg_ctx* c, bool has_u) {
    launch_apply<double, 2>(c, c->x, c->scratch[0], whole_part(c));
    GuessArgs<double> f{};
    f.begin = c->g.own_begin / 2; f.nvec = c->g.own_len / 2;
    f.b = c->b; f.ax = c->scratch[0]; f.x = c->x; f.r = c->r; f.p0 = c->p[0]; f.u = c->u;
    f.partB = c->partB; f.strideB = c->strideB; f.partG = c->guess_part; f.strideG = c->strideB; f.s_out = c->sB;
    if (has_u) hipLaunchKernelGGL((k_init_guess<double, 2, true>), dim3(c->whole.grid), dim3(kBlock), 0, c->stream, f);
    else hipLaunchKernelGGL((k_init_guess<double, 2, false>), dim3(c->whole.grid), dim3(kBlock), 0, c->stream, f);
    double* norms = c->guess_part + 2 * (size_t)c->strideB;
    hipLaunchKernelGGL(k_guess_state, dim3(1), dim3(kBlock), 0, c->stream, (const double*)c->partB, c->strideB, (const double*)c->guess_part, c->strideB,
                       c->whole.grid, c->sB, norms);
    HIPCK(hipMemcpyAsync(c->guess_norms_h, norms, sizeof(double) * 2, hipMemcpyDeviceToHost, c->stream));
    return MI355CG_OK;
}
static void launch_init_fresh(mi355cg_ctx* c, bool has_u) {
    FreshArgs<double> f{};
    f.begin = c->g.own_begin / 2; f.nvec = c->g.own_len / 2;
    f.b = c->b; f.x = c->x; f.r = c->r; f.p0 = c->p[0]; f.u = c->u;
    f.partB = c->partB; f.strideB = c->strideB; f.s_out = c->sB;
    if (has_u) hipLaunchKernelGGL((k_init_fresh<double, 2, true>), dim3(c->whole.grid), dim3(kBlock), 0, c->stream, f);
    else hipLaunchKernelGGL((k_init_fresh<double, 2, false>), dim3(c->whole.grid), dim3(kBlock), 0, c->stream, f);
}

static void launch_onchip_chunk(mi355cg_ctx* c, const IterCfg& cfg, const mi355cg_params* prm, int m) {
    OnchipArgs a{};
    a.g = c->g; a.pl = onchip_plan(c->gp.n);
    a.x = c->x; a.r = c->r; a.u = c->u;
    for (int k = 0; k < c->xsteps; ++k) a.p[k] = c->p[k];
    a.xsteps = c->xsteps;
    a.partB = c->partB; a.nB = c->nB_own; a.strideB = c->strideB;
    a.s = c->sB; a.hist = c->hist; a.rp = cfg.rp;
    a.has_u = cfg.has_u ? 1 : 0; a.u_always = cfg.rp.eps_exact_error > 0 ? 1 : 0; a.every = prm->callback_every;
    a.m = m; a.stop_req = c->stop_dev;
    const dim3 grid(1), block(a.pl.threads);
    const bool msg = cfg.rp.rule == MI355CG_RULE_MSG_MAXNORM;
#define MI355CG_OC(E) do { if (msg) hipLaunchKernelGGL((k_onchip<E, true>), grid, block, 0, c->stream, a); \
                           else hipLaunchKernelGGL((k_onchip<E, false>), grid, block, 0, c->stream, a); } while (0)
    switch (a.pl.elems) {
        case 1: MI355CG_OC(1); break;
        case 2: MI355CG_OC(2); break;
        case 4: MI355CG_OC(4); break;
        case 8: MI355CG_OC(8); break;
        case 16: MI355CG_OC(16); break;
        default: MI355CG_OC(kOnchipMaxElems); break;
    }
#undef MI355CG_OC
    c->nB_own = 1;
    ++c->onchip_launches;
}

int mi355cg_solve(mi355cg_handle c, const mi355cg_params* prm, mi355cg_iter_cb cb, void* user,
                  const volatile int* stop_flag, mi355cg_results* out) {
    if (!c || !prm) return fail(MI355CG_ERR_INVALID, "null argument");
    if (prm->rule != MI355CG_RULE_MSG_MAXNORM && prm->rule != MI355CG_RULE_REL_2NORM) return fail(MI355CG_ERR_INVALID, "unknown rule %d", prm->rule);
    if (c->is_slab) return fail(MI355CG_ERR_STATE, "this handle owns one part of a decomposed grid: use the mi355cg_team_* / mi355cg_dist_* entry points");
    HIPCK(hipSetDevice(c->device));
    const bool warm = c->guess_pending;
    c->guess_pending = false;
    c->onchip_launches = 0;
    if (c->is_csr) return solve_csr(c, prm, cb, user, stop_flag, out);
    if (c->dtype == MI355CG_F32_MIXED) return solve_mixed(c, prm, cb, user, stop_flag, out);
    if (c->mg) return solve_mg(c, prm, cb, user, stop_flag, out, warm);
    const bool msg = prm->rule == MI355CG_RULE_MSG_MAXNORM;
    IterCfg cfg0 = make_cfg(prm);
    const bool onchip = c->solve_mode == MI355CG_SOLVE_ONCHIP && cfg0.want_diag == 0;
    if (onchip) cfg0.x2 = false;
    cfg0.fold = cfg0.x2 && ensure_fold_ring(c);
    const IterCfg cfg = cfg0;
    const bool diag = cfg.want_diag != 0, fold = cfg.fold;
    c->nB_own = c->whole.grid;
    if (cfg.has_u) if (int rc = ensure_u_on_device(c)) return rc;
    if (diag || (warm && !(c->scratch[0] && c->scratch[1]))) if (int rc = ensure_scratch(c)) return rc;
    if (warm) if (int rc = ensure_guess_ws(c)) return rc;

    const auto t0 = std::chrono::steady_clock::now();
    c->events.reset(); c->ev_pairs[0].clear(); c->ev_pairs[1].clear();

    c->cur = 0; c->fcur = 0;
    if (c->qctr && c->dyn_rows > 0) HIPCK(hipMemsetAsync(c->qctr, 0, sizeof(int) * 2 * kXcds * kQueueSubs * kQueuePitch, c->stream));
    if (warm) { if (int rc = launch_init_guess(c, cfg.has_u)) return rc; }
    else launch_init_fresh(c, cfg.has_u);
    HIPCK(hipGetLastError());

    *c->stop_h = 0;
    c->stop_dev = nullptr;
    if (stop_flag) HIPCK(hipHostGetDevicePointer((void**)&c->stop_dev, c->stop_h, 0));
    auto wait_stream = [&]() -> int { return wait_stream_forwarding_stop(c, stop_flag); };
    bool polled = false;
    auto poll = [&]() -> int {
        launch_check(c, cfg, c->stream, own_partB(c));
        if (int rc = fetch_state(c, c->stream)) return rc;
        polled = true;
        return wait_stream();
    };
    *c->summary_h = CgState{};
    if (msg && (cb || warm)) {
        if (int rc = poll()) return rc;
        if (cb) cb(user, 0, DBL_MAX, c->summary_h->rmax, cfg.has_u ? c->summary_h->emax : DBL_MAX);
    }
    if (warm)
        if (const int reason = msg_stop_reason(prm, false, 0.0, c->summary_h->rmax, cfg.has_u, c->summary_h->emax)) {
            c->summary_h->done = 1; c->summary_h->converged = 1; c->summary_h->reason = reason;
        }
    if (int rc = loop_timer_begin(c, c->stream)) return rc;

    const int every = prm->callback_every;
    auto need_u = [&](int it) { return diag || cfg.rp.eps_exact_error > 0 || it == 1 || (every > 0 && it % every == 0); };
    const int sync_every = default_sync_every(prm, msg);
    int it_done = 0;
    bool interrupted = false;
    bool first_chunk = cb != nullptr || stop_flag != nullptr;
    if (std::memcmp(&c->graph_prm, prm, sizeof *prm) != 0 || c->graph_stop != (stop_flag != nullptr)) {
        clear_graphs(c); c->graph_prm = *prm; c->graph_stop = stop_flag != nullptr;
    }
    const bool graph_ok = !c->profiling && !diag &&
                          (c->use_graph == 1 || (c->use_graph < 0 && c->g.own_len < (4LL << 20) && prm->max_iterations >= 4 * sync_every));
    while (!c->summary_h->done) {
        if (stop_flag && *stop_flag) { interrupted = true; break; }
        const int m = chunk_len(prm, msg, sync_every, it_done, first_chunk);
        first_chunk = false;
        auto enqueue_chunk = [&]() -> int {
            for (int k = 0; k < m; ++k) {
                hipEvent_t e0 = nullptr;
                Buf<double> pp[kRing];
                if (fold) { pp[c->cur].borrow(c->fold_p[c->fcur]); pp[(c->cur + 1) % c->xsteps].borrow(c->fold_p[(c->fcur + 1) % c->xfold]); }
                const Buf<double>* ring = fold ? pp : c->p;
                prof_begin(c, &e0);
                launch_iteration_stencil<double, 2>(c, cfg, c->r, ring, whole_part(c), own_partB(c));
                c->cur = (c->cur + 1) % c->xsteps;
                if (fold) c->fcur = (c->fcur + 1) % c->xfold;
                prof_end(c, 0, e0);
                prof_begin(c, &e0);
                IterCfg ucfg = cfg;
                ucfg.has_u = cfg.has_u && need_u(it_done + k + 1);
                launch_iteration_update<double, 2>(c, ucfg, c->x, c->r, ring, c->u, whole_part(c), own_partA(c));
                if (fold && c->fcur == 0) launch_fold_x(c, -1, c->stream);
                prof_end(c, 1, e0);
                if (diag) {
                    launch_apply<double, 2>(c, c->x, c->scratch[0], whole_part(c));
                    hipLaunchKernelGGL((k_resid2<double>), dim3(1024), dim3(kBlock), 0, c->stream, c->g.own_begin, c->g.own_len, c->b, c->scratch[0], c->partR);
                    hipLaunchKernelGGL(k_resid2_hist, dim3(1), dim3(kBlock), 0, c->stream, c->partR, 1024, c->sB, c->hist);
                }
            }
            return MI355CG_OK;
        };
        if (onchip) {
            launch_onchip_chunk(c, cfg, prm, m);
        } else if (graph_ok && m >= 8) {
            std::vector<char> flags(m);
            for (int k = 0; k < m; ++k) flags[k] = cfg.has_u && need_u(it_done + k + 1);
            mi355cg_ctx::ChunkGraph* hit = nullptr;
            const int key = fold ? c->fcur : c->cur;
            for (auto& g : c->graphs) if (g.m == m && g.cur == key && g.flags == flags) hit = &g;
            if (!hit) {
                hipGraph_t graph = nullptr; hipGraphExec_t exec = nullptr;
                const int cur0 = c->cur, fcur0 = c->fcur;
                HIPCK(hipStreamBeginCapture(c->stream, hipStreamCaptureModeThreadLocal));
                const int rc = enqueue_chunk();
                const hipError_t e1 = hipStreamEndCapture(c->stream, &graph);
                c->cur = cur0; c->fcur = fcur0;
                if (rc) return rc;
                HIPCK(e1);
                HIPCK(hipGraphInstantiate(&exec, graph, nullptr, nullptr, 0));
                HIPCK(hipGraphDestroy(graph));
                c->graphs.push_back({m, key, flags, exec});
                hit = &c->graphs.back();
            }
            HIPCK(hipGraphLaunch(hit->exec, c->stream));
            c->cur = (c->cur + m) % c->xsteps;
            if (fold) c->fcur = (c->fcur + m) % c->xfold;
        } else {
            if (int rc = enqueue_chunk()) return rc;
        }
        HIPCK(hipGetLastError());
        if (int rc = poll()) return rc;
        const int it_now = c->summary_h->it;
        replay_callbacks(cb, user, prm, *c->summary_h, c->hist_h, it_done, it_now, cfg.has_u, diag);
        it_done = it_now;
    }
    if (int rc = loop_timer_end(c, c->stream)) return rc;
    CgState fin = *c->summary_h;
    c->stop_dev = nullptr;
    if (fin.done && fin.reason == MI355CG_STOP_INTERRUPTED) interrupted = true;
    c->cur = fin.it % c->xsteps;
    if (cfg.x2) {
        if (fold) { c->fcur = fin.it % c->xfold; if (c->fcur != 0) launch_fold_x(c, fin.it, c->stream); }
        else launch_flush_x<double, 2>(c, c->whole, c->x, c->p, fin, c->stream);
        HIPCK(hipGetLastError());
        HIPCK(hipStreamSynchronize(c->stream));
    }
    if (cfg.has_u && fin.it > 0 && !need_u(fin.it)) {
        hipLaunchKernelGGL((k_err_maxnorm<double>), dim3(1024), dim3(kBlock), 0, c->stream, c->g.own_begin, c->g.own_len, c->x, c->u, c->partR);
        HIPCK(hipGetLastError());
        HIPCK(hipMemcpyAsync(c->partR_h, c->partR, sizeof(double) * 1024, hipMemcpyDeviceToHost, c->stream));
        HIPCK(hipStreamSynchronize(c->stream));
        double m = 0; for (int i = 0; i < 1024; ++i) m = std::max(m, c->partR_h[i]);
        fin.emax = m;
    }
    c->solved = true; c->x_is_guess = false;
    prof_collect(c);
#ifdef MI355CG_WAVE_TIMING
    if (const char* path = getenv("MI355CG_WAVE_TIMING_OUT")) {
        std::vector<unsigned long long> buf(2 * kWtStamps * kWtWaves);
        HIPCK(hipMemcpyFromSymbol(buf.data(), HIP_SYMBOL(g_wave_dbg), buf.size() * sizeof(unsigned long long)));
        if (FILE* f = fopen(path, "wb")) { fwrite(buf.data(), sizeof(unsigned long long), buf.size(), f); fclose(f); }
    }
#endif
    mi355cg_results res = make_results(fin, interrupted, cfg.has_u, warm && polled ? c->guess_norms_h[0] : fin.r0norm);
    res.solve_seconds = std::chrono::duration<double>(std::chrono::steady_clock::now() - t0).count();
    HIPCK(hipEventSynchronize(c->ev_loop[1]));
    res.loop_seconds = loop_timer_seconds(c);
    if (msg && cb) cb(user, res.iterations, res.final_precision, res.final_residual_norm, res.final_error_norm);
    if (out) *out = res;
    return MI355CG_OK;
}

int mi355cg_get_solution(mi355cg_handle c, double* x) {
    if (!c || !x) return fail(MI355CG_ERR_INVALID, "null argument");
    if (c->x_is_guess) return fail(MI355CG_ERR_STATE, "an initial guess was set after the last solve: x holds the guess, not a solution");
    if (!c->solved) return fail(MI355CG_ERR_STATE, "no solve has run on this handle");
    HIPCK(hipSetDevice(c->device));
    return download_packed<double>(c, c->x, x);
}
int mi355cg_get_recursive_residual(mi355cg_handle c, double* r) {
    if (!c || !r) return fail(MI355CG_ERR_INVALID, "null argument");
    if (c->x_is_guess) return fail(MI355CG_ERR_STATE, "an initial guess was set after the last solve: r is not the residual of x");
    if (!c->solved) return fail(MI355CG_ERR_STATE, "no solve has run on this handle");
    HIPCK(hipSetDevice(c->device));
    return download_packed<double>(c, c->r, r);
}
int mi355cg_get_true_residual(mi355cg_handle c, double* out) {
    if (!c || !out) return fail(MI355CG_ERR_INVALID, "null argument");
    if (c->is_slab) return fail(MI355CG_ERR_STATE, "this handle owns one part of a decomposed grid: use the mi355cg_team_* / mi355cg_dist_* entry points");
    if (c->x_is_guess) return fail(MI355CG_ERR_STATE, "an initial guess was set after the last solve: x holds the guess, not a solution");
    if (!c->solved) return fail(MI355CG_ERR_STATE, "no solve has run on this handle");
    HIPCK(hipSetDevice(c->device));
    if (int rc = ensure_scratch(c)) return rc;
    if (c->is_csr) launch_csr_spmv(c, c->x, c->scratch[0], nullptr, nullptr, nullptr);
    else launch_apply<double, 2>(c, c->x, c->scratch[0], whole_part(c));
    hipLaunchKernelGGL((k_sub<double>), dim3(flat_grid(c->g.own_len)), dim3(kBlock), 0, c->stream, c->g.own_begin, c->g.own_len, c->scratch[0], c->b, c->scratch[1]);
    HIPCK(hipGetLastError());
    return download_packed<double>(c, c->scratch[1], out);
}

static int guess_check(mi355cg_ctx* c) {
    if (!c) return fail(MI355CG_ERR_INVALID, "null handle");
    if (c->is_csr) return fail(MI355CG_ERR_INVALID, "an initial guess needs the grid operator's start (r0 = b - A x0): a CSR handle has none");
    if (c->is_slab) return fail(MI355CG_ERR_INVALID, "an initial guess is single-GPU only: this handle owns one part of a decomposed grid");
    if (c->dtype != MI355CG_F64) return fail(MI355CG_ERR_INVALID, "an initial guess is fp64 only: this handle was created with MI355CG_F32_MIXED");
    return MI355CG_OK;
}

int mi355cg_set_initial_guess(mi355cg_handle c, const double* x0) {
    if (int rc = guess_check(c)) return rc;
    if (!x0) { c->guess_pending = false; return MI355CG_OK; }
    HIPCK(hipSetDevice(c->device));
    c->x_is_guess = true;
    if (int rc = upload_packed<double>(c, x0, c->x)) return rc;
    c->guess_pending = true;
    return MI355CG_OK;
}

int mi355cg_set_initial_guess_device(mi355cg_handle c, const double* x0_dev) {
    if (int rc = guess_check(c)) return rc;
    if (!x0_dev) return fail(MI355CG_ERR_INVALID, "null argument");
    HIPCK(hipSetDevice(c->device));
    c->x_is_guess = true;
    hipLaunchKernelGGL((k_unpack<double>), dim3(flat_grid(c->pk_len)), dim3(kBlock), 0, c->stream, c->pg, x0_dev, c->x);
    HIPCK(hipGetLastError());
    HIPCK(hipStreamSynchronize(c->stream));
    c->guess_pending = true;
    return MI355CG_OK;
// ... 62 lines not shown
        if (c->is_slab) HIPCK(hipDeviceSynchronize());
        if (c->pk_len > 0) hipLaunchKernelGGL((k_pack<double>), dim3(flat_grid(c->pk_len)), dim3(kBlock), 0, c->stream, c->pg, (const double*)c->x, x_dev);
        HIPCK(hipGetLastError());
    }
    HIPCK(hipStreamSynchronize(c->stream));
    return MI355CG_OK;
}

static void launch_step_rhs(mi355cg_ctx* c, double sigma, double theta) {
    StepRhsArgs a{};
    a.g = c->g;
    a.A0 = c->gp.A; a.xk = c->gp.x_k; a.yk = c->gp.y_k;
    a.sigma = sigma; a.theta = theta; a.c1 = (1.0 - theta) / theta;
    a.u = c->x; a.rhs = c->b; a.out = c->step_b;
    a.tiles_per_row = (c->g.N + kStepTileCols) / kStepTileCols;
    a.tiles = (long long)(c->g.N - 1) * a.tiles_per_row;
    const int grid = (int)std::min<long long>(a.tiles, 1 << 20);
    if (theta < 1.0) hipLaunchKernelGGL((k_step_rhs<true>), dim3(grid), dim3(kBlock), 0, c->stream, a);
    else hipLaunchKernelGGL((k_step_rhs<false>), dim3(grid), dim3(kBlock), 0, c->stream, a);
}

int mi355cg_time_steps(mi355cg_handle c, const mi355cg_params* prm, double tau, double theta, int nsteps,
                       const volatile int* stop_flag, mi355cg_results* out, int* steps_done) {
    if (!c || !prm || !out || !steps_done) return fail(MI355CG_ERR_INVALID, "null argument");
    if (int rc = shift_check(c)) return rc;
    if (!std::isfinite(tau) || !(tau > 0.0)) return fail(MI355CG_ERR_INVALID, "time step %g rejected: tau must be finite and > 0", tau);
    if (!(theta > 0.0 && theta <= 1.0)) return fail(MI355CG_ERR_INVALID, "theta %g rejected: the scheme needs 0 < theta <= 1", theta);
    if (nsteps < 0) return fail(MI355CG_ERR_INVALID, "nsteps %d rejected: it must be >= 0", nsteps);
    if (prm->rule != MI355CG_RULE_MSG_MAXNORM && prm->rule != MI355CG_RULE_REL_2NORM) return fail(MI355CG_ERR_INVALID, "unknown rule %d", prm->rule);
    if (prm->diagnostics) return fail(MI355CG_ERR_INVALID, "the stepper has no callbacks: diagnostics must be 0");
    if (prm->use_true_solution) return fail(MI355CG_ERR_INVALID, "a step has no exact solution: use_true_solution must be 0");
    const double sigma = 1.0 / (theta * tau);
    if (!std::isfinite(sigma)) return fail(MI355CG_ERR_INVALID, "time step %g rejected: 1 / (theta tau) is not finite", tau);
    if (nsteps == 0) { *steps_done = 0; return MI355CG_OK; }
    if (!c->guess_pending) return fail(MI355CG_ERR_STATE, "no starting state: set it with mi355cg_set_initial_guess* or mi355cg_use_solution_as_initial_guess");
    *steps_done = 0;
    HIPCK(hipSetDevice(c->device));
    if (!c->step_b) {
        if (int rc = Buf<double>::device_zeroed(c->step_b, c->storage_len)) return rc;
        HIPCK(hipDeviceSynchronize());
    }
    if (int rc = mi355cg_set_shift(c, sigma)) return rc;
    for (int k = 0; k < nsteps; ++k) {
        if (k > 0) { c->x_is_guess = true; c->guess_pending = true; }
        launch_step_rhs(c, sigma, theta);
        HIPCK(hipGetLastError());
        std::swap(c->b, c->step_b);
        const int rc = mi355cg_solve(c, prm, nullptr, nullptr, stop_flag, &out[k]);
        std::swap(c->b, c->step_b);
        if (rc) return rc;
        if (!out[k].converged) break;
        ++*steps_done;
    }
    return MI355CG_OK;
}

int mi355cg_set_profiling(mi355cg_handle c, int enable) {
    if (!c) return fail(MI355CG_ERR_INVALID, "null handle");
    c->profiling = enable != 0;
    return MI355CG_OK;
}
int mi355cg_get_kernel_time(mi355cg_handle c, int kernel, double* avg_ms, long long* launches) {
    if (!c || kernel < 0 || kernel > 1) return fail(MI355CG_ERR_INVALID, "bad argument");
    if (avg_ms) *avg_ms = c->kernel_ms[kernel];
    if (launches) *launches = c->kernel_launches[kernel];
    return MI355CG_OK;
}
int mi355cg_get_layout(mi355cg_handle c, long long* padded_len, int* pitch_bottom, int* pitch_upper,
                       int* grid_stencil, int* grid_update, int* rows_per_item) {
    if (!c) return fail(MI355CG_ERR_INVALID, "null handle");
    if (padded_len) *padded_len = c->g.own_len;
    if (pitch_bottom) *pitch_bottom = c->g.Pb;
    if (pitch_upper) *pitch_upper = c->g.Pu;
    if (grid_stencil) *grid_stencil = c->whole.grid;
    if (grid_update) *grid_update = c->whole.grid;
    if (rows_per_item) *rows_per_item = c->whole.ty;
    return MI355CG_OK;
}

int mi355cg_get_xfold(mi355cg_handle c, int* depth, int* extra_buffers) {
    if (!c) return fail(MI355CG_ERR_INVALID, "null handle");
    if (depth) *depth = c->xfold;
    if (extra_buffers) *extra_buffers = c->fold_extra;
    return MI355CG_OK;
}

int mi355cg_set_solve_mode(mi355cg_handle c, int mode) {
    if (!c) return fail(MI355CG_ERR_INVALID, "null handle");
    if (mode != MI355CG_SOLVE_LAUNCHES && mode != MI355CG_SOLVE_ONCHIP)
        return fail(MI355CG_ERR_INVALID, "unknown solve mode %d (MI355CG_SOLVE_LAUNCHES = 0, MI355CG_SOLVE_ONCHIP = 1)", mode);
    if (mode == MI355CG_SOLVE_ONCHIP) if (const char* why = onchip_refusal(c)) return fail(MI355CG_ERR_INVALID, "%s", why);
    if (mode == c->solve_mode) return MI355CG_OK;
    HIPCK(hipSetDevice(c->device));
    HIPCK(hipStreamSynchronize(c->stream));
    clear_graphs(c);
    c->solve_mode = mode;
    return MI355CG_OK;
}
int mi355cg_get_solve_mode(mi355cg_handle c, int* mode, long long* onchip_launches_last_solve) {
    if (!c) return fail(MI355CG_ERR_INVALID, "null handle");
    if (mode) *mode = c->solve_mode;
    if (onchip_launches_last_solve) *onchip_launches_last_solve = c->onchip_launches;
    return MI355CG_OK;
}
int mi355cg_onchip_plan(int n, int* threads, int* lds_bytes, int* elems_per_thread) {
    if (!onchip_supported(n))
        return fail(MI355CG_ERR_INVALID, "grid %d rejected: the on-chip solve takes even n from 6 to %d", n, kOnchipMaxN);
    const OnchipPlan pl = onchip_plan(n);
    if (threads) *threads = pl.threads;
    if (lds_bytes) *lds_bytes = pl.lds_bytes;
    if (elems_per_thread) *elems_per_thread = pl.elems;
    return MI355CG_OK;
}

int mi355cg_mg_levels(int n, int* levels, int* coarsest_n) {
    std::vector<int> ns;
    if (int rc = mg_shape(MI355CG_PRECOND_MG, n, &ns)) return rc;
    if (levels) *levels = (int)ns.size();
    if (coarsest_n) *coarsest_n = ns.back();
    return MI355CG_OK;
}

int mi355cg_mg_hierarchy(int kind, int n, int max_levels, int* levels, int* level_n) {
    if (max_levels < 0 || (max_levels > 0 && !level_n)) return fail(MI355CG_ERR_INVALID, "level_n must hold max_levels >= 0 entries");
    std::vector<int> ns;
    if (int rc = mg_shape(kind, n, &ns)) return rc;
    if (levels) *levels = (int)ns.size();
    for (int l = 0; l < (int)ns.size() && l < max_levels; ++l) level_n[l] = ns[l];
    return MI355CG_OK;
}

int mi355cg_set_preconditioner(mi355cg_handle c, int kind) { return mi355cg_set_preconditioner_ex(c, kind, MI355CG_CYCLE_F64); }

int mi355cg_set_preconditioner_ex(mi355cg_handle c, int kind, int cycle) {
    if (!c) return fail(MI355CG_ERR_INVALID, "null handle");
    if (kind != MI355CG_PRECOND_NONE && kind != MI355CG_PRECOND_MG && kind != MI355CG_PRECOND_MG_ANY)
        return fail(MI355CG_ERR_INVALID, "unknown preconditioner kind %d (MI355CG_PRECOND_NONE = 0, MI355CG_PRECOND_MG = 1, "
                    "MI355CG_PRECOND_MG_ANY = 2)", kind);
    HIPCK(hipSetDevice(c->device));
    if (kind == MI355CG_PRECOND_NONE) {
        mg_batch_free(c);
        eig_free(c);
        if (c->mg) { HIPCK(hipStreamSynchronize(c->stream)); c->mg.reset(); }
        return MI355CG_OK;
    }
    if (c->is_csr) return fail(MI355CG_ERR_INVALID, "the multigrid preconditioner needs the grid operator: a CSR handle has no grid");
    if (c->is_slab) return fail(MI355CG_ERR_INVALID, "the multigrid preconditioner is single-GPU only: this handle owns one part of a decomposed grid");
    if (c->dtype != MI355CG_F64) return fail(MI355CG_ERR_INVALID, "the multigrid preconditioner is fp64 only: this handle was created with MI355CG_F32_MIXED");
    if (c->solve_mode == MI355CG_SOLVE_ONCHIP)
        return fail(MI355CG_ERR_INVALID, "this handle is in the on-chip solve mode, which runs plain CG: mi355cg_set_solve_mode(h, MI355CG_SOLVE_LAUNCHES) first");
    std::vector<int> ns;
    if (int rc = mg_shape(kind, c->gp.n, &ns)) return rc;
    if (cycle != MI355CG_CYCLE_F64 && cycle != MI355CG_CYCLE_F32)
        return fail(MI355CG_ERR_INVALID, "unknown V-cycle precision %d (MI355CG_CYCLE_F64 = 0, MI355CG_CYCLE_F32 = 1)", cycle);
    if (cycle == MI355CG_CYCLE_F32 && c->smoother != MI355CG_SMOOTHER_JACOBI)
        return fail(MI355CG_ERR_INVALID, "the fp32 V-cycle smooths with point Jacobi only: this handle has line smoother %d "
                    "(mi355cg_set_smoother(h, MI355CG_SMOOTHER_JACOBI) first)", c->smoother);
    mg_batch_free(c);
    eig_free(c);
    if (c->mg && c->mg->cycle == cycle) { c->mg->kind = kind; return MI355CG_OK; }
    if (c->mg) HIPCK(hipStreamSynchronize(c->stream));
    return mg_build(c, kind, c->mg, cycle);
}

int mi355cg_set_smoother(mi355cg_handle c, int smoother) {
    if (!c) return fail(MI355CG_ERR_INVALID, "null handle");
// ... 640 lines not shown
```

### iterative_solvers_amd/solver.py

```python
from __future__ import annotations

import ctypes as C
import enum
import sys
from dataclasses import dataclass, field
from typing import Callable, Optional

import numpy as np

from . import _capi

DBL_MAX = sys.float_info.max
BATCH_MAX = _capi.BATCH_MAX


class StopCriterion(enum.IntEnum):
    ITERATIONS = 0
    PRECISION = 1
    RESIDUAL = 2
    EXACT_ERROR = 3
    INTERRUPTED = 4


_STOP_TEXT = {
# ... 304 lines not shown
        return np.ascontiguousarray(v)

    def eigs(self, nev: int, block: int, tol: float, max_iterations: int, x, stop_flag: Optional[C.c_int] = None):
        nev, block = int(nev), int(block)
        on_device = not isinstance(x, np.ndarray)
        if on_device:
            if not (type(x).__module__.split(".")[0] == "torch" and hasattr(x, "data_ptr")):
                raise ValueError(f"a start block is a NumPy array or a CUDA torch tensor, not {type(x).__name__}")
            import torch
            if not x.is_cuda:
                raise ValueError("a torch start block must be in device memory (a CPU tensor: pass tensor.numpy())")
            if x.dtype != torch.float64:
                raise ValueError(f"start block has dtype {x.dtype}, expected torch.float64")
            if x.device.index != self._device:
                raise ValueError(f"start block is on {x.device}, the handle on device {self._device}")
        elif x.dtype != np.float64:
            raise ValueError(f"start block has dtype {x.dtype}, expected float64")
        if tuple(x.shape) != (block, self.size):
            raise ValueError(f"start block has shape {tuple(x.shape)}, expected ({block}, {self.size})")
        lam, res = np.zeros(max(block, 1)), np.zeros(max(block, 1))
        out = _capi.EigResults()
        sp = C.cast(C.pointer(stop_flag), C.c_void_p) if stop_flag is not None else None
        if on_device:
            v = x.contiguous().clone()
            torch.cuda.current_stream(x.device).synchronize()
            rc = self._lib.mi355cg_eigs_device(self._h, nev, block, float(tol), int(max_iterations), v.data_ptr(), lam.ctypes.data,
                                               res.ctypes.data, sp, C.byref(out))
        else:
            v = np.array(x, dtype=np.float64, order="C", copy=True)
            rc = self._lib.mi355cg_eigs(self._h, nev, block, float(tol), int(max_iterations), v.ctypes.data, lam.ctypes.data,
                                        res.ctypes.data, sp, C.byref(out))
        if rc == _capi.ERR_INVALID:
            raise ValueError(self._lib.mi355cg_last_error().decode())
        _capi.check(rc)
        return lam[:block], v, res[:block], out

    def eigs_release(self):
        _capi.check(self._lib.mi355cg_eigs_release(self._h))

    def block_gram(self, a, b, rows=None, cols=None):
        a = self._check_block(a, self.size, _capi.EIG_BASIS_MAX, "a")
        b = self._check_block(b, self.size, _capi.EIG_BASIS_MAX, "b")
        ia = None if rows is None else np.ascontiguousarray(rows, dtype=np.int32)
        ib = None if cols is None else np.ascontiguousarray(cols, dtype=np.int32)
        out = np.empty((a.shape[0] if ia is None else ia.size, b.shape[0] if ib is None else ib.size))
        rc = self._lib.mi355cg_block_gram_indexed(self._h, a.shape[0], a.ctypes.data, 0 if ia is None else ia.size,
                                                  None if ia is None else ia.ctypes.data, b.shape[0], b.ctypes.data,
                                                  0 if ib is None else ib.size, None if ib is None else ib.ctypes.data, out.ctypes.data)
        if rc == _capi.ERR_INVALID:
            raise ValueError(self._lib.mi355cg_last_error().decode())
        _capi.check(rc)
        return out

    def block_combine(self, s, coef):
        s = self._check_block(s, self.size, _capi.EIG_BASIS_MAX, "s")
        coef = np.ascontiguousarray(coef, dtype=np.float64)
        if coef.ndim != 2 or coef.shape[0] != s.shape[0] or not 1 <= coef.shape[1] <= _capi.EIG_BLOCK_MAX:
            raise ValueError(f"coef has shape {tuple(coef.shape)}, expected ({s.shape[0]}, 1 .. {_capi.EIG_BLOCK_MAX})")
        y = np.empty((coef.shape[1], self.size))
        rc = self._lib.mi355cg_block_combine(self._h, s.shape[0], s.ctypes.data, coef.shape[1], coef.ctypes.data, y.ctypes.data)
        if rc == _capi.ERR_INVALID:
            raise ValueError(self._lib.mi355cg_last_error().decode())
        _capi.check(rc)
        return y

    def setup_on_device(self):
        _capi.check(self._lib.mi355cg_setup_on_device(self._h))

    def set_profiling(self, on: bool):
        _capi.check(self._lib.mi355cg_set_profiling(self._h, 1 if on else 0))

    def kernel_time(self, kernel: int):
        ms, n = C.c_double(), C.c_longlong()
        _capi.check(self._lib.mi355cg_get_kernel_time(self._h, kernel, C.byref(ms), C.byref(n)))
        return ms.value, n.value

    def layout(self):
        L = C.c_longlong()
        v = [C.c_int() for _ in range(5)]
        _capi.check(self._lib.mi355cg_get_layout(self._h, C.byref(L), *[C.byref(i) for i in v]))
        fold, extra = C.c_int(), C.c_int()
        if hasattr(self._lib, "mi355cg_get_xfold"):
            _capi.check(self._lib.mi355cg_get_xfold(self._h, C.byref(fold), C.byref(extra)))
        return {"padded_len": L.value, "pitch_bottom": v[0].value, "pitch_upper": v[1].value,
                "grid_stencil": v[2].value, "grid_update": v[3].value, "rows_per_item": v[4].value,
                "x_fold": fold.value, "x_fold_buffers": extra.value}


def default_params(rule: int) -> _capi.Params:
    p = _capi.Params()
    _capi.load().mi355cg_default_params(C.byref(p), rule)
    return p


def mg_levels(n: int):
    L, nc = C.c_int(), C.c_int()
    lib = _capi.load()
    rc = lib.mi355cg_mg_levels(int(n), C.byref(L), C.byref(nc))
    if rc == _capi.ERR_INVALID:
        raise ValueError(lib.mi355cg_last_error().decode())
    _capi.check(rc)
    return L.value, nc.value


def mg_hierarchy(n: int, kind: int = _capi.PRECOND_MG_ANY):
    L = C.c_int()
    buf = (C.c_int * 64)()
    lib = _capi.load()
    rc = lib.mi355cg_mg_hierarchy(int(kind), int(n), len(buf), C.byref(L), buf)
    if rc == _capi.ERR_INVALID:
        raise ValueError(lib.mi355cg_last_error().decode())
    _capi.check(rc)
    return tuple(buf[:L.value])


def onchip_plan(n: int):
    t, lds, e = C.c_int(), C.c_int(), C.c_int()
    lib = _capi.load()
    rc = lib.mi355cg_onchip_plan(int(n), C.byref(t), C.byref(lds), C.byref(e))
    if rc == _capi.ERR_INVALID:
        raise ValueError(lib.mi355cg_last_error().decode())
    _capi.check(rc)
    return {"threads": t.value, "lds_bytes": lds.value, "elems_per_thread": e.value}


def rayleigh_ritz(g, h):
    g = np.ascontiguousarray(g, dtype=np.float64)
    h = np.ascontiguousarray(h, dtype=np.float64)
    if g.ndim != 2 or g.shape[0] != g.shape[1] or h.shape != g.shape:
        raise ValueError(f"G and H are square matrices of one size, not {tuple(g.shape)} and {tuple(h.shape)}")
    k = g.shape[0]
    theta, coef = np.empty(max(k, 1)), np.empty((max(k, 1), max(k, 1)))
    lib = _capi.load()
    rc = lib.mi355cg_rayleigh_ritz(k, g.ctypes.data, h.ctypes.data, theta.ctypes.data, coef.ctypes.data)
    if rc == _capi.ERR_INVALID:
        raise ValueError(lib.mi355cg_last_error().decode())
    _capi.check(rc)
    return theta, coef


class MatrixFreeSystem:

    def __init__(self, m, n, a, b, c, d, device: int = 0, dtype: int = _capi.F64):
        self.n, self.m = n, m
        self.domain = (a, b, c, d)
        self._handle = _Handle(n, m, a, b, c, d, dtype=dtype, device=device)

    def get_rhs(self) -> np.ndarray: return self._handle.rhs()
    def get_true_solution_vector(self) -> np.ndarray: return self._handle.true_solution()
    def size(self) -> int: return self._handle.size

    def apply(self, x, y=None) -> np.ndarray:
        out = self._handle.apply(x)
        if y is not None:
            y[...] = out
            return y
        return out

    def __mul__(self, x): return self.apply(x)

    def set_preconditioner(self, kind: int, cycle: int = _capi.CYCLE_F64):
        self._handle.set_preconditioner(kind, cycle)

    def preconditioner_info(self):
        return self._handle.preconditioner_info()

    def set_solve_mode(self, mode: int):
        self._handle.set_solve_mode(mode)

# ... 291 lines not shown
```

Before: 8609 iters/s.

## Lean cold start: skip zero-x init pass and fold x only at the end

With a zero initial guess, the full init pass is replaced by a norm-only kernel over b. The first iteration's stencil treats p as zero and its update reads r from b, and the first x fold skips loading x. Separately, the x fold for the final partial window runs on device inside the poll after the check, and the history copy is dropped when no callback needs it. This saves a few full-vector passes and a sync per solve, which is small against 2641 iterations, at the cost of extra kernel variants and more graph keys.

```diff
diff --git a/include/mi355cg.h b/include/mi355cg.h
--- a/include/mi355cg.h
+++ b/include/mi355cg.h
@@ -154,6 +154,7 @@
 int  mi355cg_get_layout(mi355cg_handle h, long long *padded_len, int *pitch_bottom, int *pitch_upper,
                         int *grid_stencil, int *grid_update, int *rows_per_item);
 int  mi355cg_get_xfold(mi355cg_handle h, int *depth, int *extra_buffers);
+int  mi355cg_get_cold_start(mi355cg_handle h, int *lean);
 
 #define MI355CG_SOLVE_LAUNCHES 0
 #define MI355CG_SOLVE_ONCHIP   1
diff --git a/iterative_solvers_amd/_capi.py b/iterative_solvers_amd/_capi.py
--- a/iterative_solvers_amd/_capi.py
+++ b/iterative_solvers_amd/_capi.py
@@ -28,7 +28,7 @@
     "mi355cg_team_set_profiling", "mi355cg_team_phase_times", "mi355cg_team_describe", "mi355cg_setup_on_device", "mi355cg_team_setup_on_device", "mi355cg_debug_plan",
     "mi355cg_team_set_dtype", "mi355cg_set_preconditioner", "mi355cg_apply_preconditioner", "mi355cg_mg_levels",
     "mi355cg_mg_hierarchy", "mi355cg_set_preconditioner_ex", "mi355cg_preconditioner_info",
-    "mi355cg_solve_batch", "mi355cg_solve_batch_device", "mi355cg_batch_release", "mi355cg_get_xfold",
+    "mi355cg_solve_batch", "mi355cg_solve_batch_device", "mi355cg_batch_release", "mi355cg_get_xfold", "mi355cg_get_cold_start",
     "mi355cg_set_initial_guess", "mi355cg_set_initial_guess_device", "mi355cg_use_solution_as_initial_guess",
     "mi355cg_solve_batch_from", "mi355cg_solve_batch_device_from",
     "mi355cg_set_shift", "mi355cg_get_shift", "mi355cg_time_steps", "mi355cg_get_solution_device",
@@ -213,6 +213,8 @@
         L.mi355cg_solve_many_info.argtypes = [H, C.c_int, IP, IP, LLP]
     if hasattr(L, "mi355cg_get_xfold"):
         L.mi355cg_get_xfold.argtypes = [H, IP, IP]
+    if hasattr(L, "mi355cg_get_cold_start"):
+        L.mi355cg_get_cold_start.argtypes = [H, IP]
     _lib = L
     return L
 
diff --git a/iterative_solvers_amd/csrc/cg_kernels.h b/iterative_solvers_amd/csrc/cg_kernels.h
--- a/iterative_solvers_amd/csrc/cg_kernels.h
+++ b/iterative_solvers_amd/csrc/cg_kernels.h
@@ -542,9 +542,10 @@
     return A;
 }
 
-template <typename T, int VEC, bool FUSED, bool MSG, int DEPTH, bool NOAP, bool GC, bool TEAM, bool QUEUE>
+template <typename T, int VEC, bool FUSED, bool MSG, int DEPTH, bool NOAP, bool GC, bool TEAM, bool QUEUE, bool FIRST = false>
 __global__ __launch_bounds__(kBlock) void k_stencil(const StencilArgs<T> a) {
     static_assert(DEPTH >= 1 && DEPTH <= 3, "the compute cursor takes its item from the fetch cursor: DEPTH <= rows fetched per item (>= 3)");
+    static_assert(!FIRST || (FUSED && !TEAM && !MSG && !GC), "FIRST: the single-context REL_2NORM iteration launch only");
     typedef typename VecOf<T, VEC>::type vec_t;
     __shared__ double lds[2 * kWaves];
     const Geom& g = a.g;
@@ -597,10 +598,12 @@
         int ve = own ? F.ve_own : kOob;
         if (!f_have) { vo = kOob; ve = kOob; }
         Raw w;
-        w.p = buf_load<vec_t>(rs_p, vo, f_so);
+        if constexpr (FIRST) { for (int j = 0; j < VEC; ++j) w.p[j] = (T)0; }
+        else w.p = buf_load<vec_t>(rs_p, vo, f_so);
         if (FUSED) w.r = buf_load<vec_t>(rs_r, vo, f_so);
         else for (int j = 0; j < VEC; ++j) w.r[j] = (T)0;
-        w.pe = buf_load<T>(rs_p, ve, f_so);
+        if constexpr (FIRST) w.pe = (T)0;
+        else w.pe = buf_load<T>(rs_p, ve, f_so);
         if (FUSED) w.re = buf_load<T>(rs_r, ve, f_so); else w.re = (T)0;
         f_so += row_step<T>(g, f_y); ++f_y; ++f_idx;
         return w;
@@ -917,6 +920,40 @@
     }
 }
 
+__global__ __launch_bounds__(kBlock) void k_norm_fresh(const FreshArgs<double> a) {
+    typedef VecOf<double, 2>::type vec_t;
+    __shared__ double lds[2 * kWaves];
+    dd s_rr = dd_zero();
+    double s_rmax = 0;
+    const long long stride = (long long)gridDim.x * kBlock;
+    const vec_t* __restrict__ B = reinterpret_cast<const vec_t*>(a.b);
+    const long long end = a.begin + a.nvec;
+    auto take = [&](const vec_t& bv) {
+#pragma unroll
+        for (int j = 0; j < 2; ++j) {
+            const double rd = bv[j];
+            dd_acc_prod(s_rr, rd, rd);
+            s_rmax = fmax(s_rmax, fabs(rd));
+        }
+    };
+    long long i = a.begin + (long long)blockIdx.x * kBlock + threadIdx.x;
+    for (; i + 3 * stride < end; i += 4 * stride) {
+        const vec_t b0 = B[i], b1 = B[i + stride], b2 = B[i + 2 * stride], b3 = B[i + 3 * stride];
+        take(b0); take(b1); take(b2); take(b3);
+    }
+    for (; i < end; i += stride) take(B[i]);
+    const dd t_rr = block_reduce_dd(s_rr, lds);
+    const double t_rmax = block_reduce<true>(s_rmax, lds);
+    if (threadIdx.x == 0) {
+        const int b = blockIdx.x, st = a.strideB;
+        a.partB[FB_RR * st + b] = t_rr.hi; a.partB[(FB_RR + FB_LO) * st + b] = t_rr.lo;
+        a.partB[FB_D2 * st + b] = 0.0; a.partB[(FB_D2 + FB_LO) * st + b] = 0.0;
+        a.partB[FB_E2 * st + b] = 0.0; a.partB[(FB_E2 + FB_LO) * st + b] = 0.0;
+        a.partB[FB_RMAX * st + b] = t_rmax; a.partB[FB_DMAX * st + b] = 0.0; a.partB[FB_EMAX * st + b] = 0.0;
+        if (blockIdx.x == 0) { *a.s_out = CgState{}; a.s_out->first = 1; }
+    }
+}
+
 template <typename T>
 struct GuessArgs {
     long long begin, nvec;
@@ -1002,11 +1039,13 @@
     QueueSpec dq;
     double* fold_alpha;
     int fold_mask;
+    const T* rin;
 };
 
-template <typename T, int VEC, int XM, bool HAS_U, int DEPTH, bool DESC, bool TEAM, bool QUEUE>
+template <typename T, int VEC, int XM, bool HAS_U, int DEPTH, bool DESC, bool TEAM, bool QUEUE, bool FIRST = false>
 __global__ __launch_bounds__(kBlock) void k_update_st(const UpdateStArgs<T> a) {
     static_assert(DEPTH >= 1 && DEPTH <= 3, "see k_stencil");
+    static_assert(!FIRST || (XM == 0 && !TEAM), "FIRST: the single-context launch that leaves x to k_fold_x only");
     typedef typename VecOf<T, VEC>::type vec_t;
     __shared__ double lds[2 * kWaves];
     const Geom& g = a.g;
@@ -1043,7 +1082,8 @@
         if (QUEUE && dq) dq_ticket = queue_take(dq, lane);
         F = item_addr<T, VEC, DESC>(g, u, lane);
         rs_p = make_rsrc(a.p + F.base_el);
-        rs_r = make_rsrc(a.r + F.base_el);
+        if constexpr (FIRST) rs_r = make_rsrc(a.rin + F.base_el);
+        else rs_r = make_rsrc(a.r + F.base_el);
         rs_x = make_rsrc(XM != 0 ? a.x + F.base_el : a.p + F.base_el);
 #pragma unroll
         for (int i = 0; i < NP; ++i) rs_pp[i] = make_rsrc(a.pprev[i] + F.base_el);
@@ -1303,6 +1343,7 @@
 }
 
 constexpr int kFoldMax = 32;
+constexpr int kFoldAtEnd = -2;
 struct FoldTable { const double* p[kFoldMax]; double alpha[kFoldMax]; };
 struct FoldArgs {
     long long begin, nvec;
@@ -1311,6 +1352,7 @@
     const CgState* s;
     int mask;
     int flush_it;
+    int cold;
 };
 template <int NS, bool NT>
 __device__ inline void fold_block(VecOf<double, 2>::type& xv, const FoldTable* tab, int k0, int mask, long long i) {
@@ -1332,15 +1374,19 @@
     typedef VecOf<double, 2>::type vec_t;
     const int it = a.flush_it >= 0 ? a.flush_it : scalar_load(&a.s->it);
     int n = it & a.mask;
-    if (a.flush_it < 0) {
+    if (a.flush_it == kFoldAtEnd) {
+        if (!scalar_load(&a.s->done)) return;
+    } else if (a.flush_it < 0) {
         if (scalar_load(&a.s->done) || n != 0 || it == 0) return;
         n = a.mask + 1;
     }
     if (n == 0) return;
+    const bool from_zero = a.cold != 0 && it == n;
     vec_t* __restrict__ X = reinterpret_cast<vec_t*>(a.x);
     const long long stride = (long long)gridDim.x * kBlock, end = a.begin + a.nvec;
     for (long long i = a.begin + (long long)blockIdx.x * kBlock + threadIdx.x; i < end; i += stride) {
-        vec_t xv = X[i];
+        vec_t xv = {0.0, 0.0};
+        if (!from_zero) xv = X[i];
         int k = it - n + 1;
         for (; k + 8 <= it + 1; k += 8) fold_block<8, NT>(xv, a.tab, k, a.mask, i);
         if (k + 4 <= it + 1) { fold_block<4, NT>(xv, a.tab, k, a.mask, i); k += 4; }
diff --git a/iterative_solvers_amd/csrc/mi355cg.hip b/iterative_solvers_amd/csrc/mi355cg.hip
--- a/iterative_solvers_amd/csrc/mi355cg.hip
+++ b/iterative_solvers_amd/csrc/mi355cg.hip
@@ -23,6 +23,7 @@
 #include <memory>
 #include <string>
 #include <thread>
+#include <type_traits>
 #include <vector>
 
 using namespace mi355cg;
@@ -216,8 +217,9 @@
     int fcur = 0;
     int fold_grid = 0;
     bool fold_nt = true;
-
-    struct ChunkGraph { int m, cur; std::vector<char> flags; hipGraphExec_t exec; };
+    bool lean_start = false, fold_at_end = false;
+
+    struct ChunkGraph { int m, cur; std::vector<char> flags; hipGraphExec_t exec; int lead; };
     std::vector<ChunkGraph> graphs;
     mi355cg_params graph_prm{};
     bool graph_stop = false;
@@ -401,7 +403,8 @@
 struct IterCfg { RuleParams rp; int want_diag; bool has_u; bool x2 = false; bool fold = false; };
 
 template <typename T, int VEC>
-void launch_iteration_stencil(mi355cg_ctx* c, const IterCfg& cfg, const T* r, const Buf<T> p[kRing], const Where& w, const PartSrc& pb, const FlagSpec* fl = nullptr) {
+void launch_iteration_stencil(mi355cg_ctx* c, const IterCfg& cfg, const T* r, const Buf<T> p[kRing], const Where& w, const PartSrc& pb, const FlagSpec* fl = nullptr,
+                              bool first = false) {
     if (w.plan->wl.nitems == 0) return;
     StencilArgs<T> a{};
     a.g = kernel_geom<T, VEC>(c); a.tab = item_tab(*w.plan);
@@ -415,6 +418,13 @@
     const dim3 grid(w.plan->grid), block(kBlock);
     const bool msg = cfg.rp.rule == MI355CG_RULE_MSG_MAXNORM, gc = c->has_gc, d3 = c->depth == 3;
     const bool team = pb.rec.mbox != nullptr || (fl && fl->part), queue = a.dq.mine != nullptr;
+    if constexpr (VEC == 2 && std::is_same<T, double>::value) {
+        if (first) {
+            if (queue) hipLaunchKernelGGL((k_stencil<T, VEC, true, false, 3, true, false, false, true, true>), grid, block, 0, w.stream, a);
+            else hipLaunchKernelGGL((k_stencil<T, VEC, true, false, 3, true, false, false, false, true>), grid, block, 0, w.stream, a);
+            return;
+        }
+    }
 #define MI355CG_ST(MSG, D, GC) do { if (team) hipLaunchKernelGGL((k_stencil<T, VEC, true, MSG, D, true, GC, true, VEC == 2>), grid, block, 0, w.stream, a); \
                                     else if (VEC == 2 && queue) hipLaunchKernelGGL((k_stencil<T, VEC, true, MSG, D, true, GC, false, VEC == 2>), grid, block, 0, w.stream, a); \
                                     else hipLaunchKernelGGL((k_stencil<T, VEC, true, MSG, D, true, GC, false, false>), grid, block, 0, w.stream, a); } while (0)
@@ -428,7 +438,8 @@
 }
 
 template <typename T, int VEC>
-void launch_iteration_update(mi355cg_ctx* c, const IterCfg& cfg, T* x, T* r, const Buf<T> p[kRing], const T* u, const Where& w, const PartSrc& pa, const FlagSpec* fl = nullptr) {
+void launch_iteration_update(mi355cg_ctx* c, const IterCfg& cfg, T* x, T* r, const Buf<T> p[kRing], const T* u, const Where& w, const PartSrc& pa, const FlagSpec* fl = nullptr,
+                             const T* first_rin = nullptr) {
     if (w.plan->wl.nitems == 0) return;
     UpdateStArgs<T> a{};
     a.g = kernel_geom<T, VEC>(c); a.tab = item_tab(*w.plan);
@@ -444,6 +455,14 @@
     const dim3 grid(w.plan->grid), block(kBlock);
     const bool d3 = c->depth == 3 && !(cfg.x2 && c->cur == 0 && c->xsteps == 8);
     const bool team = pa.rec.mbox != nullptr || (fl && fl->part), queue = a.dq.mine != nullptr;
+    if constexpr (VEC == 2 && std::is_same<T, double>::value) {
+        if (first_rin) {
+            a.rin = first_rin;
+            if (queue) hipLaunchKernelGGL((k_update_st<T, VEC, 0, false, 3, true, false, true, true>), grid, block, 0, w.stream, a);
+            else hipLaunchKernelGGL((k_update_st<T, VEC, 0, false, 3, true, false, false, true>), grid, block, 0, w.stream, a);
+            return;
+        }
+    }
 #define MI355CG_UST_D(XM, HASU, D) do { if (team) hipLaunchKernelGGL((k_update_st<T, VEC, XM, HASU, D, true, true, VEC == 2>), grid, block, 0, w.stream, a); \
                                         else if (VEC == 2 && queue) hipLaunchKernelGGL((k_update_st<T, VEC, XM, HASU, D, true, false, VEC == 2>), grid, block, 0, w.stream, a); \
                                         else hipLaunchKernelGGL((k_update_st<T, VEC, XM, HASU, D, true, false, false>), grid, block, 0, w.stream, a); } while (0)
@@ -481,10 +500,10 @@
                        kernel_geom<T, VEC>(c), item_tab(plan), x, f);
 }
 
-void launch_fold_x(const mi355cg_ctx* c, int flush_it, hipStream_t stream) {
+void launch_fold_x(const mi355cg_ctx* c, int flush_it, hipStream_t stream, bool cold = false) {
     FoldArgs a{};
     a.begin = c->g.own_begin / 2; a.nvec = c->g.own_len / 2;
-    a.x = c->x; a.tab = c->fold_tab; a.s = c->sB; a.mask = c->xfold - 1; a.flush_it = flush_it;
+    a.x = c->x; a.tab = c->fold_tab; a.s = flush_it == kFoldAtEnd ? c->summary : c->sB; a.mask = c->xfold - 1; a.flush_it = flush_it; a.cold = cold ? 1 : 0;
     const long long one_shot = (a.nvec + kBlock - 1) / kBlock;
     const int grid = (int)std::max<long long>(1, c->fold_grid > 0 ? std::min<long long>(c->fold_grid, one_shot) : one_shot);
     if (c->fold_nt) hipLaunchKernelGGL((k_fold_x<true>), dim3(grid), dim3(kBlock), 0, stream, a);
@@ -639,9 +658,9 @@
     c->events.reset();
 }
 
-int fetch_state(mi355cg_ctx* c, hipStream_t st) {
+int fetch_state(mi355cg_ctx* c, hipStream_t st, bool with_hist = true) {
     HIPCK(hipMemcpyAsync(c->summary_h, c->summary, sizeof(CgState), hipMemcpyDeviceToHost, st));
-    HIPCK(hipMemcpyAsync(c->hist_h, c->hist, sizeof(HistEntry) * kHist, hipMemcpyDeviceToHost, st));
+    if (with_hist) HIPCK(hipMemcpyAsync(c->hist_h, c->hist, sizeof(HistEntry) * kHist, hipMemcpyDeviceToHost, st));
     return MI355CG_OK;
 }
 int wait_stream_forwarding_stop(mi355cg_ctx* c, const volatile int* stop_flag) {
@@ -1867,6 +1886,8 @@
         }
         c->fold_grid = std::max(0, env_int("MI355CG_XFOLD_GRID", 0));
         c->fold_nt = env_int("MI355CG_XFOLD_NT", 1) != 0;
+        { const char* v = getenv("MI355CG_COLD_START"); c->lean_start = !(v && std::strcmp(v, "pass") == 0); }
+        { const char* v = getenv("MI355CG_END_FOLD"); c->fold_at_end = !(v && std::strcmp(v, "host") == 0); }
     }
     Buf<double>* vecs[] = {&c->x, &c->r, &c->p[0], &c->p[1], &c->ap, &c->b, &c->u, &c->p[2], &c->p[3], &c->p[4], &c->p[5], &c->p[6], &c->p[7]};
     for (int k = 0; k < 7 + (c->xsteps - 2); ++k) if ((rc = Buf<double>::device_zeroed(*vecs[k], L))) return cleanup();
@@ -2094,6 +2115,13 @@
     else hipLaunchKernelGGL((k_init_fresh<double, 2, false>), dim3(c->whole.grid), dim3(kBlock), 0, c->stream, f);
 }
 
+static void launch_norm_fresh(mi355cg_ctx* c) {
+    FreshArgs<double> f{};
+    f.begin = c->g.own_begin / 2; f.nvec = c->g.own_len / 2;
+    f.b = c->b; f.partB = c->partB; f.strideB = c->strideB; f.s_out = c->sB;
+    hipLaunchKernelGGL(k_norm_fresh, dim3(c->whole.grid), dim3(kBlock), 0, c->stream, f);
+}
+
 static void launch_onchip_chunk(mi355cg_ctx* c, const IterCfg& cfg, const mi355cg_params* prm, int m) {
     OnchipArgs a{};
     a.g = c->g; a.pl = onchip_plan(c->gp.n);
@@ -2140,6 +2168,8 @@
     cfg0.fold = cfg0.x2 && ensure_fold_ring(c);
     const IterCfg cfg = cfg0;
     const bool diag = cfg.want_diag != 0, fold = cfg.fold;
+    const bool lean = fold && !warm && c->lean_start && c->depth == 3;
+    const bool fold_at_end = fold && c->fold_at_end;
     c->nB_own = c->whole.grid;
     if (cfg.has_u) if (int rc = ensure_u_on_device(c)) return rc;
     if (diag || (warm && !(c->scratch[0] && c->scratch[1]))) if (int rc = ensure_scratch(c)) return rc;
@@ -2151,6 +2181,7 @@
     c->cur = 0; c->fcur = 0;
     if (c->qctr && c->dyn_rows > 0) HIPCK(hipMemsetAsync(c->qctr, 0, sizeof(int) * 2 * kXcds * kQueueSubs * kQueuePitch, c->stream));
     if (warm) { if (int rc = launch_init_guess(c, cfg.has_u)) return rc; }
+    else if (lean) launch_norm_fresh(c);
     else launch_init_fresh(c, cfg.has_u);
     HIPCK(hipGetLastError());
 
@@ -2159,9 +2190,11 @@
     if (stop_flag) HIPCK(hipHostGetDevicePointer((void**)&c->stop_dev, c->stop_h, 0));
     auto wait_stream = [&]() -> int { return wait_stream_forwarding_stop(c, stop_flag); };
     bool polled = false;
+    const bool want_hist = !fold_at_end || (cb != nullptr && (msg || diag));
     auto poll = [&]() -> int {
         launch_check(c, cfg, c->stream, own_partB(c));
-        if (int rc = fetch_state(c, c->stream)) return rc;
+        if (fold_at_end) launch_fold_x(c, kFoldAtEnd, c->stream, lean);
+        if (int rc = fetch_state(c, c->stream, want_hist)) return rc;
         polled = true;
         return wait_stream();
     };
@@ -2182,6 +2215,7 @@
     int it_done = 0;
     bool interrupted = false;
     bool first_chunk = cb != nullptr || stop_flag != nullptr;
+    bool loop_closed = false;
     if (std::memcmp(&c->graph_prm, prm, sizeof *prm) != 0 || c->graph_stop != (stop_flag != nullptr)) {
         clear_graphs(c); c->graph_prm = *prm; c->graph_stop = stop_flag != nullptr;
     }
@@ -2198,15 +2232,16 @@
                 if (fold) { pp[c->cur].borrow(c->fold_p[c->fcur]); pp[(c->cur + 1) % c->xsteps].borrow(c->fold_p[(c->fcur + 1) % c->xfold]); }
                 const Buf<double>* ring = fold ? pp : c->p;
                 prof_begin(c, &e0);
-                launch_iteration_stencil<double, 2>(c, cfg, c->r, ring, whole_part(c), own_partB(c));
+                const bool first = lean && it_done + k == 0;
+                launch_iteration_stencil<double, 2>(c, cfg, first ? c->b.get() : c->r.get(), ring, whole_part(c), own_partB(c), nullptr, first);
                 c->cur = (c->cur + 1) % c->xsteps;
                 if (fold) c->fcur = (c->fcur + 1) % c->xfold;
                 prof_end(c, 0, e0);
                 prof_begin(c, &e0);
                 IterCfg ucfg = cfg;
                 ucfg.has_u = cfg.has_u && need_u(it_done + k + 1);
-                launch_iteration_update<double, 2>(c, ucfg, c->x, c->r, ring, c->u, whole_part(c), own_partA(c));
-                if (fold && c->fcur == 0) launch_fold_x(c, -1, c->stream);
+                launch_iteration_update<double, 2>(c, ucfg, c->x, c->r, ring, c->u, whole_part(c), own_partA(c), nullptr, first ? c->b.get() : nullptr);
+                if (fold && c->fcur == 0) launch_fold_x(c, -1, c->stream, lean);
                 prof_end(c, 1, e0);
                 if (diag) {
                     launch_apply<double, 2>(c, c->x, c->scratch[0], whole_part(c));
@@ -2223,7 +2258,8 @@
             for (int k = 0; k < m; ++k) flags[k] = cfg.has_u && need_u(it_done + k + 1);
             mi355cg_ctx::ChunkGraph* hit = nullptr;
             const int key = fold ? c->fcur : c->cur;
-            for (auto& g : c->graphs) if (g.m == m && g.cur == key && g.flags == flags) hit = &g;
+            const int lead = !lean ? 0 : it_done == 0 ? 2 : 1;
+            for (auto& g : c->graphs) if (g.m == m && g.cur == key && g.flags == flags && g.lead == lead) hit = &g;
             if (!hit) {
                 hipGraph_t graph = nullptr; hipGraphExec_t exec = nullptr;
                 const int cur0 = c->cur, fcur0 = c->fcur;
@@ -2235,7 +2271,7 @@
                 HIPCK(e1);
                 HIPCK(hipGraphInstantiate(&exec, graph, nullptr, nullptr, 0));
                 HIPCK(hipGraphDestroy(graph));
-                c->graphs.push_back({m, key, flags, exec});
+                c->graphs.push_back({m, key, flags, exec, lead});
                 hit = &c->graphs.back();
             }
             HIPCK(hipGraphLaunch(hit->exec, c->stream));
@@ -2245,21 +2281,28 @@
             if (int rc = enqueue_chunk()) return rc;
         }
         HIPCK(hipGetLastError());
+        if (fold_at_end) { if (int rc = loop_timer_end(c, c->stream)) return rc; loop_closed = true; }
         if (int rc = poll()) return rc;
         const int it_now = c->summary_h->it;
         replay_callbacks(cb, user, prm, *c->summary_h, c->hist_h, it_done, it_now, cfg.has_u, diag);
         it_done = it_now;
     }
-    if (int rc = loop_timer_end(c, c->stream)) return rc;
+    if (!loop_closed) if (int rc = loop_timer_end(c, c->stream)) return rc;
     CgState fin = *c->summary_h;
     c->stop_dev = nullptr;
     if (fin.done && fin.reason == MI355CG_STOP_INTERRUPTED) interrupted = true;
     c->cur = fin.it % c->xsteps;
     if (cfg.x2) {
-        if (fold) { c->fcur = fin.it % c->xfold; if (c->fcur != 0) launch_fold_x(c, fin.it, c->stream); }
+        bool launched = true;
+        if (fold) {
+            c->fcur = fin.it % c->xfold;
+            launched = c->fcur != 0 && !(fold_at_end && fin.done);
+            if (launched) launch_fold_x(c, fin.it, c->stream, lean);
+            if (lean && fin.it == 0) { launch_init_fresh(c, cfg.has_u); launched = true; }
+        }
         else launch_flush_x<double, 2>(c, c->whole, c->x, c->p, fin, c->stream);
         HIPCK(hipGetLastError());
-        HIPCK(hipStreamSynchronize(c->stream));
+        if (launched) HIPCK(hipStreamSynchronize(c->stream));
     }
     if (cfg.has_u && fin.it > 0 && !need_u(fin.it)) {
         hipLaunchKernelGGL((k_err_maxnorm<double>), dim3(1024), dim3(kBlock), 0, c->stream, c->g.own_begin, c->g.own_len, c->x, c->u, c->partR);
@@ -2488,6 +2531,13 @@
     if (!c) return fail(MI355CG_ERR_INVALID, "null handle");
     if (depth) *depth = c->xfold;
     if (extra_buffers) *extra_buffers = c->fold_extra;
+    return MI355CG_OK;
+}
+
+int mi355cg_get_cold_start(mi355cg_handle c, int* lean) {
+    if (!c || !lean) return fail(MI355CG_ERR_INVALID, "null argument");
+    *lean = (c->lean_start && c->xfold != 0 && c->depth == 3 && !c->is_csr && !c->is_slab && c->dtype == MI355CG_F64 && !c->mg &&
+             c->solve_mode != MI355CG_SOLVE_ONCHIP) ? 1 : 0;
     return MI355CG_OK;
 }
 
diff --git a/iterative_solvers_amd/solver.py b/iterative_solvers_amd/solver.py
--- a/iterative_solvers_amd/solver.py
+++ b/iterative_solvers_amd/solver.py
@@ -410,9 +410,12 @@
         fold, extra = C.c_int(), C.c_int()
         if hasattr(self._lib, "mi355cg_get_xfold"):
             _capi.check(self._lib.mi355cg_get_xfold(self._h, C.byref(fold), C.byref(extra)))
+        lean = C.c_int()
+        if hasattr(self._lib, "mi355cg_get_cold_start"):
+            _capi.check(self._lib.mi355cg_get_cold_start(self._h, C.byref(lean)))
         return {"padded_len": L.value, "pitch_bottom": v[0].value, "pitch_upper": v[1].value,
                 "grid_stencil": v[2].value, "grid_update": v[3].value, "rows_per_item": v[4].value,
-                "x_fold": fold.value, "x_fold_buffers": extra.value}
+                "x_fold": fold.value, "x_fold_buffers": extra.value, "cold_start": "lean" if lean.value else "pass"}
 
 
 def default_params(rule: int) -> _capi.Params:
```

After: 8609 iters/s, median of 2. No clear change (+0.0%).
